# maxjiang216/corintho-ai

Hardware: AMD Instinct MI355X
Metric: self-play games/sec at 400 sims/move (higher is better)
Workload: dtype f32(f16x3)

## Files before the change

corintho_ai_amd/csrc/kernels.h:

```cpp
#pragma once
#include "mcts.h"

CO_CONST int32_t CO_SPACE_SYM[8][16] = CO_SPACE_SYM_INIT;
CO_CONST int32_t CO_MOVE_SYM[8][96] = CO_MOVE_SYM_INIT;

#ifdef CO_EMU
#define CO_K3_WAVES 1
#define CO_K3_WAVE_IN_BLOCK 0
#define CO_K3_BOUNDS
#else
#define CO_K3_BOUNDS __launch_bounds__(CO_K3_WPB * 64)
#define CO_K3_WAVES CO_K3_WPB
#define CO_K3_WAVE_IN_BLOCK (CO_K3_WPB > 1 ? __builtin_amdgcn_readfirstlane((int)(threadIdx.x >> 6)) : 0)
#endif
CO_K3_BOUNDS CO_KERNEL co_k_mcts_step(EngineParams P) {
  const int i = CO_BLOCK_IDX * CO_K3_WAVES + CO_K3_WAVE_IN_BLOCK;
  const int g = P.pool_lo + i;
  if (i < P.pool_n && g < P.num_games) co_mcts_step_wave(P, g);
}

CO_DEV int co_game_active(const EngineParams &P, int g, const GameCtl &gc, int tp) {
  if (gc.done) return 0;
  if (P.pcfg) return tp == CO_TO_PLAY_EVERY_MODEL || P.pcfg[2 * g + gc.to_play].model_id == tp;
  if (tp == 0 || tp == 1) return gc.to_play == (tp + gc.parity) % 2;
  return 1;
}

CO_KERNEL co_k_scan(EngineParams P) {
  int G = P.num_games;
  const int tp = P.arena_state ? P.arena_state[P.scan_phase == 0 ? CO_AS_NEXT : CO_AS_MODEL] : P.to_play;
  int chunk = (G + CO_WAVE - 1) / CO_WAVE;
  LV(int, csum);
  LV(int, nd);
  LV(int, er);
  FOR_LANES {
    int s = 0, notdone = 0, err = 0;
    for (int i = 0; i < chunk; ++i) {
      int g = lane * chunk + i;
      if (g < G) {
        GameCtl gc = P.games[g];
        if (co_game_active(P, g, gc, tp)) s += gc.n_pending;
        notdone += !gc.done;
        err |= gc.error;
      }
    }
    L(csum) = s;
    L(nd) = notdone;
    L(er) = err != 0;
  }
  int not_done = WAVE_SUM_I32(nd);
  int any_error = WAVE_BALLOT(er) != 0;
  WAVE_SHARED(int, cbase, CO_WAVE + 1);
  FOR_LANES { cbase[lane + 1] = L(csum); }
  WAVE_SYNC();
  int run = 0;
  LV(int, mybase);
  FOR_LANES { L(mybase) = 0; }
  for (int l = 0; l < CO_WAVE; ++l) {
    int v = cbase[l + 1];
    FOR_LANES {
      if (lane == l) L(mybase) = run;
    }
    run += v;
  }
  FOR_LANES {
    int s = L(mybase);
    for (int i = 0; i < chunk; ++i) {
      int g = lane * chunk + i;
      if (g < G) {
        GameCtl gc = P.games[g];
        P.req_offset[g] = s;
        if (co_game_active(P, g, gc, tp)) s += gc.n_pending;
      }
    }
    if (lane == 0 && P.read_offset) {
      int offset = 0;
      P.read_offset[0] = 0;
      for (int i = 1; i < G; ++i) {
        if (co_game_active(P, i, P.games[i], tp)) offset += P.games[i - 1].n_pending;
        P.read_offset[i] = offset;
      }
    }
    if (lane == 0) {
      P.req_offset[G] = run;
      P.all_done[0] = not_done == 0;
      if (P.ctl) {
        P.ctl[CO_CTL_ROWS] = run;
        P.ctl[CO_CTL_ALL_DONE] = not_done == 0;
        P.ctl[CO_CTL_ANY_ERROR] = any_error;
        P.ctl[CO_CTL_NOT_DONE] = not_done;
      }
      if (P.row_counter && (!P.arena_state || P.scan_phase == 1)) P.row_counter[0] += (unsigned long long)run;
      if (P.arena_state) {
        if (P.scan_phase == 0) {
          P.arena_state[CO_AS_MODEL] = tp;
        } else {
          P.arena_state[CO_AS_ROWS + (tp == 0 ? 1 : 0)] = run;
          P.arena_state[CO_AS_ROWS + (tp == 0 ? 0 : 1)] = 0;
          if (not_done != 0 && run == 0) {
            P.arena_state[CO_AS_NEXT] = 1 - tp;
            P.arena_state[CO_AS_EMPTY] += 1;
          } else {
            P.arena_state[CO_AS_NEXT] = tp;
            P.arena_state[CO_AS_EMPTY] = 0;
          }
        }
      }
    }
  }
}

CO_KERNEL co_k_compact(EngineParams P) {
  int g = CO_BLOCK_IDX;
  if (g >= P.num_games) return;
  GameCtl gc = P.games[g];
  if (!co_game_active(P, g, gc, P.arena_state ? P.arena_state[CO_AS_MODEL] : P.to_play)) return;
  int n = gc.n_pending;
  const float *src = P.req + (size_t)g * P.searches_per_eval * CO_STATE_STRIDE;
  float *dst = P.nn_in + (size_t)P.req_offset[g] * CO_STATE_STRIDE;
  int total = n * CO_STATE_STRIDE;
  FOR_LANES {
    for (int i = lane; i < total; i += CO_WAVE) dst[i] = src[i];
  }
  if (P.nn_in70) {
    float *d70 = P.nn_in70 + (size_t)P.req_offset[g] * CO_GAME_STATE_SIZE;
    int t70 = n * CO_GAME_STATE_SIZE;
    FOR_LANES {
      for (int i = lane; i < t70; i += CO_WAVE) d70[i] = src[(i / CO_GAME_STATE_SIZE) * CO_STATE_STRIDE + i % CO_GAME_STATE_SIZE];
    }
  }
}

CO_KERNEL co_k_expand_rows(const float *in70, float *out80, int rows, int nblocks) {
  FOR_LANES {
    int total = rows * CO_STATE_STRIDE;
    for (int i = CO_BLOCK_IDX * CO_WAVE + lane; i < total; i += CO_WAVE * nblocks) {
      int r = i / CO_STATE_STRIDE, c = i % CO_STATE_STRIDE;
      out80[i] = c < CO_GAME_STATE_SIZE ? in70[(size_t)r * CO_GAME_STATE_SIZE + c] : 0.0f;
    }
  }
}

#define CO_HOST_ROWS_FLOAT ((CO_BLOCK_IDX * CO_WAVES_PER_BLOCK + CO_WAVE_IN_BLOCK) * CO_WAVE + lane)
CO_KERNEL co_k_host_rows_out(const float *req, const int32_t *in_idx, const uint32_t *count, int cap_rows, float *out70) {
  const uint32_t have = count[0];
  const int rows = (int)(have < (uint32_t)cap_rows ? have : (uint32_t)cap_rows);
  const int total = cap_rows * CO_GAME_STATE_SIZE;
  FOR_LANES {
    const int e = CO_HOST_ROWS_FLOAT;
    if (e < total) {
      const int r = e / CO_GAME_STATE_SIZE, c = e - r * CO_GAME_STATE_SIZE;
      out70[e] = r < rows ? req[(size_t)(in_idx ? in_idx[r] : r) * CO_STATE_STRIDE + c] : 0.0f;
    }
  }
}
CO_KERNEL co_k_host_rows_in(const float *evals, const float *probs, const int32_t *out_idx, const uint32_t *count, int rows,
                            float *d_eval, float *d_probs, int eval_stride, int probs_stride) {
  const uint32_t have = count ? count[0] : (uint32_t)rows;
  const int total = (int)(have < (uint32_t)rows ? have : (uint32_t)rows) * (1 + CO_NUM_MOVES);
  FOR_LANES {
    const int e = CO_HOST_ROWS_FLOAT;
    if (e < total) {
      const int r = e / (1 + CO_NUM_MOVES), c = e - r * (1 + CO_NUM_MOVES);
      const size_t o = (size_t)(out_idx ? out_idx[r] : r);
      if (c == 0) d_eval[o * (size_t)eval_stride] = evals[r];
      else d_probs[o * (size_t)probs_stride + c - 1] = probs[(size_t)r * CO_NUM_MOVES + c - 1];
    }
  }
}

CO_KERNEL co_k_write_samples(EngineParams P, int n_games, const int32_t *sample_offset, const int32_t *meta, float *game_states,
                             float *eval_samples, float *prob_samples) {
  int g = CO_BLOCK_IDX;
  if (g >= n_games) return;
  const int n = meta[g] & 255, result = meta[g] >> 8;
  size_t off = (size_t)sample_offset[g];
  const float *smp = P.samples + (size_t)g * CO_MAX_PLIES * CO_SAMPLE_FLOATS;
  for (int i = n - 1; i >= 0; --i) {
    const float evaluation = co_sample_outcome(result, n, i);
    const float *st = smp + (size_t)i * CO_SAMPLE_FLOATS;
    const float *pol = st + CO_GAME_STATE_SIZE;
    for (int k = 0; k < CO_NUM_SYMMETRIES; ++k) {
      float *gs = game_states + ((off + i) * CO_NUM_SYMMETRIES + k) * CO_GAME_STATE_SIZE;
      float *ps = prob_samples + ((off + i) * CO_NUM_SYMMETRIES + k) * CO_NUM_MOVES;
      FOR_LANES {
        gs[lane] = st[CO_SPACE_SYM[k][lane / 4] * 4 + lane % 4];
        if (lane < CO_GAME_STATE_SIZE - 64) gs[64 + lane] = st[64 + lane];
        ps[lane] = pol[CO_MOVE_SYM[k][lane]];
        if (lane < CO_NUM_MOVES - 64) ps[64 + lane] = pol[CO_MOVE_SYM[k][64 + lane]];
        if (lane == 0) eval_samples[(off + i) * CO_NUM_SYMMETRIES + k] = evaluation;
      }
    }
  }
}

CO_KERNEL co_k_pack_samples(EngineParams P, int n_games, const int32_t *sample_offset, const int32_t *meta, float *state_policy,
                            float *outcome) {
  int g = CO_BLOCK_IDX;
  if (g >= n_games) return;
  const int n = meta[g] & 255, result = meta[g] >> 8;
  size_t off = (size_t)sample_offset[g];
  const float *smp = P.samples + (size_t)g * CO_MAX_PLIES * CO_SAMPLE_FLOATS;
  int total = n * CO_SAMPLE_FLOATS;
  FOR_LANES {
    for (int i = lane; i < total; i += CO_WAVE) state_policy[off * CO_SAMPLE_FLOATS + i] = smp[i];
    for (int i = lane; i < n; i += CO_WAVE) outcome[off + i] = co_sample_outcome(result, n, i);
  }
}

CO_KERNEL co_k_rules_batch(const uint64_t *boards, const uint32_t *metas, int n, uint32_t *masks, int32_t *lines) {
  int i = CO_BLOCK_IDX;
  if (i >= n) return;
  uint32_t lm[3];
  CoLanes K;
  co_lanes_init(K);
  int l = co_legal_moves(boards[i], metas[i], lm, K);
  FOR_LANES {
    if (lane < 3) masks[i * 3 + lane] = lm[lane];
    if (lane == 0) lines[i] = l;
  }
}

CO_KERNEL co_k_domove_batch(uint64_t *boards, uint32_t *metas, const int32_t *moves, int n, float *states) {
  int i = CO_BLOCK_IDX;
  if (i >= n) return;
  uint64_t b = boards[i];
  uint32_t m = metas[i];
  CoLanes K;
  co_lanes_init(K);
  if (moves[i] >= 0) co_do_move(&b, &m, moves[i], K);
  WAVE_SYNC();
  FOR_LANES {
    if (lane == 0) {
      boards[i] = b;
      metas[i] = m;
    }
  }
  co_write_state(b, m, states + (size_t)i * CO_STATE_STRIDE);
}

CO_KERNEL co_k_rules_rows(uint64_t *boards, uint32_t *metas, const int32_t *moves, int n, uint32_t *masks) {
  const int base = CO_BLOCK_IDX * 4;
  LV(uint32_t, blo);
  LV(uint32_t, bhi);
  LV(uint32_t, mt);
  LV(int, on);
  FOR_LANES {
    const int i = base + (lane >> 4);
    L(on) = i < n;
    uint64_t b = L(on) ? boards[i] : 0ull;
    uint32_t m = L(on) ? metas[i] : 0u;
    if (L(on) && moves[i] >= 0) co_do_move_lane(&b, &m, moves[i]);
    L(blo) = (uint32_t)b;
    L(bhi) = (uint32_t)(b >> 32);
    L(mt) = m;
  }
  LV(uint32_t, o0);
  LV(uint32_t, o1);
  LV(uint32_t, o2);
  WG_SHARED(uint32_t, lb, CO_LB_WORDS);
  co_line_breakers_to_lds(lb);
  LV(int, lines);
  co_legal_moves_rows(blo, bhi, mt, on, o0, o1, o2, lines, lb);
  FOR_LANES {
    const int i = base + (lane >> 4);
    if (L(on) && (lane & 15) == 0) {
      boards[i] = (uint64_t)L(blo) | ((uint64_t)L(bhi) << 32);
      metas[i] = L(mt);
      masks[i * 3 + 0] = L(o0);
      masks[i * 3 + 1] = L(o1);
      masks[i * 3 + 2] = L(o2);
    }
  }
}

CO_KERNEL co_k_rng_draw(uint32_t *mt, int32_t *idx_io, int n, int chunk, uint32_t *out) {
  int idx = idx_io[0];
  int done = 0;
  while (done < n) {
    int cnt = n - done < chunk ? n - done : chunk;
    LV(uint32_t, r);
    CO_MT_DRAW(mt, idx, cnt, r);
    FOR_LANES {
      if (lane < cnt) out[done + lane] = L(r);
    }
    done += cnt;
  }
  FOR_LANES {
    if (lane == 0) idx_io[0] = idx;
  }
}

CO_KERNEL co_k_fp_probe(const float *in, int n, float *out) {
  FOR_LANES {
    int i = CO_BLOCK_IDX * CO_WAVE + lane;
    if (i < n) {
      const float *x = in + (size_t)i * 8;
      float c_puct = x[0], visits = x[1], eval = x[2], p9 = x[3], denom = x[4], cv = x[5], sum = x[6], eps = x[7];
      float v_sqrt = (float)((double)c_puct * co_sqrt_f64((double)visits));
      float prob = p9 * denom;
      float pv = prob * v_sqrt;
      int icv = (int)cv;
      double a, b;
      if ((float)icv == cv && icv >= 1 && icv < 32768) {
        a = co_div_small(-(double)eval, cv);
        b = co_div_small((double)pv, cv + 1.0f);
      } else {
        a = -1.0 * (double)eval / (double)cv;
        b = (double)pv / ((double)cv + 1.0);
      }
      float one_minus = (float)1 - eps;
      float *o = out + (size_t)i * 8;
      o[0] = v_sqrt;
      o[1] = (float)(a + b);
      o[2] = pv;
      o[3] = (float)(1.0 / (double)sum * (double)one_minus);
      o[4] = (float)(1.0 / (double)sum * (double)eps);
      o[5] = 511.0f / sum;
      o[6] = (float)(1.0 / (double)(float)(int)cv);
      float xq = p9 * (511.0f / sum);
      float fl = __builtin_truncf(xq);
      int q = (int)fl;
      if (xq - fl >= 0.5f) q += 1;
      o[7] = (float)q;
    }
  }
}
```

corintho_ai_amd/csrc/pools.h:

```cpp
#pragma once
#include <algorithm>
#include <string>
#include <vector>

#include "host.h"
#include "kernels.h"

#define CO_MAX_POOLS 4
#define CO_POOL_POLL 16

struct RunStats {
  double mcts_ms = 0, nn_ms = 0, pack_ms = 0;
  int64_t mcts_launches = 0, nn_launches = 0, nn_rows = 0;
  double mcts_timed_ms = 0, nn_timed_ms = 0, pack_timed_ms = 0;
  int64_t timed_launches = 0, nn_timed_rows = 0;
  int64_t nn_rows_evaluated = 0;
  int64_t steps_cut = 0, step_budget_last = 0;
  int64_t cache_clears = 0;

  void estimate_device_times(bool with_pack) {
    if (timed_launches == 0) return;
    mcts_ms = mcts_timed_ms * (double)mcts_launches / (double)timed_launches;
    nn_ms = nn_timed_ms * (double)nn_launches / (double)timed_launches;
    if (with_pack) pack_ms = pack_timed_ms * (double)nn_launches / (double)timed_launches;
  }
};

static void launch_mcts_step(const EngineParams &e, int n, rt_stream_t s) {
  RT_LAUNCH(co_k_mcts_step, (n + CO_K3_WAVES - 1) / CO_K3_WAVES, CO_WAVE * CO_K3_WAVES, s, e);
}

struct CacheTable {
  DevBuf<uint32_t> hdr;
  DevBuf<float> val;
  DevBuf<uint32_t> done;
  size_t entries = 0;

  void create(int eval_cache, int R, int spe, rt_stream_t s) {
    size_t want = (size_t)R * 8192, n = 1;
    while (n < want) n <<= 1;
    const size_t per = 16 + CO_CACHE_VAL_FLOATS * 4;
    while (n > 1024 && n * per > rt_mem_free() / 6) n >>= 1;
    if (eval_cache > 0) {
      n = (size_t)1 << (eval_cache < 6 ? 6 : eval_cache > 30 ? 30 : eval_cache);
      if (n * per > rt_mem_free() / 2)
        throw CaError(CA_ERR_ARG, "ca_config.eval_cache: a table of 2^" + std::to_string(eval_cache) +
                                          " entries does not fit in the free device memory");
    }
    entries = n;
    hdr.alloc(n * 4, s);
    val.alloc((n + (size_t)R * spe) * CO_CACHE_VAL_FLOATS, s);
    done.alloc(CO_MAX_POOLS, s);
  }
  void release() {
    hdr.release();
    val.release();
    done.release();
    entries = 0;
  }
  void empty(rt_stream_t s, bool new_generation) {
    rt_memset(hdr.p, 0, entries * 16, s);
    if (new_generation) rt_memset(done.p, 0, 4 * CO_MAX_POOLS, s);
  }
};

struct Pool {
  Stream st;
  int lo = 0, n = 0, row_base = 0;
  bool finished = false;
  int idle = 0;
  int running = 0;
  Event ev[2][4];
  Event polled[2];
  int launched[2] = {0, 0};
  int word_iter[2] = {0, 0};
  int first_start = 0;
  int timed[2] = {0, 0};
  struct Seen {
    unsigned long long pack;
    unsigned long long cuts;
    uint32_t evaluated;
  };
  Pinned<Seen> seen;
  unsigned long long cuts_seen = 0;
  DevBuf<int32_t> in_idx, out_idx;
  DevBuf<uint32_t> count;
  DevBuf<unsigned long long> totals;
  EvalCache cache = {};
  double c_inserted_est = 0;
  Event quiet;

  void create(int p, int npools, int R, int spe) {
    st.create();
    lo = (int)((int64_t)R * p / npools);
    n = (int)((int64_t)R * (p + 1) / npools) - lo;
    row_base = lo * spe;
    for (int w = 0; w < 2; ++w) {
      for (auto &e : ev[w]) e.create();
      polled[w].create();
    }
    seen.alloc(2);
    quiet.create();
  }

  void attach(const CacheTable &table, int p, int spe) {
    const size_t rows = (size_t)n * spe;
    in_idx.alloc(rows, st);
    out_idx.alloc(rows, st);
    count.alloc(2 * CO_CACHE_COUNT_STRIDE, st);
    totals.alloc(CO_CACHE_TOTALS, st);
    cache.hdr = table.hdr.p;
    cache.val = table.val.p;
    cache.mask = (uint32_t)(table.entries - 1);
    cache.scratch_base = (uint32_t)row_base;
    cache.pool_bits = (uint32_t)p << CO_CACHE_POOL_SHIFT;
    cache.done = table.done.p;
    cache.in_idx = in_idx.p;
    cache.out_idx = out_idx.p;
    cache.count = count.p;
    cache.totals = totals.p;
    rt_sync(st);
  }

  void begin_run(unsigned long long cuts, int first) {
    cuts_seen = cuts;
    finished = false;
    running = n;
    idle = 0;
    launched[0] = launched[1] = 0;
    timed[0] = timed[1] = 0;
    word_iter[0] = word_iter[1] = 0;
    first_start = first;
  }
};

struct FusedRun {
  CacheTable table;
  std::vector<Pool> pools;
  bool cache_clean = false;
  bool host_stepped = false;

  EngineParams run_params;
  unsigned long long *work_counter = nullptr;
  float *nn_eval = nullptr, *nn_probs = nullptr;
  CoNet *net = nullptr;
  RunStats *stats = nullptr;
  rt_stream_t stream = {};
  int npools = 0, spe = 0;
  static constexpr int poll = CO_POOL_POLL;
  int32_t iteration = 0;
  int window = 0, in_window = 0, parity = 0;
  long long guard_from = -1;
  std::string failure;

  void create(int n, int R, int eval_cache) {
    pools.clear();
    table.release();
    pools.resize(n);
    for (int p = 0; p < n; ++p) {
      Pool &q = pools[p];
      q.create(p, n, R, spe);
      if (eval_cache >= 0) {
        if (p == 0) table.create(eval_cache, R, spe, q.st);
        q.attach(table, p, spe);
      }
    }
    cache_clean = true;
  }
  void release() {
    pools.clear();
    table.release();
  }

  std::vector<unsigned long long> read_work_counters() {
    std::vector<unsigned long long> wc((size_t)CO_WC_WORDS * CO_MAX_POOLS);
    rt_d2h(wc.data(), work_counter, wc.size() * 8, stream);
    rt_sync(stream);
    return wc;
  }

  bool begin(bool mid_generation) {
    const bool cache_clean_now = table.entries && !cache_clean;
    if (cache_clean_now) {
      table.empty(pools[0].st, true);
      for (auto &q : pools) {
        if (!mid_generation) {
          rt_memset(q.count.p, 0, 2 * CO_CACHE_COUNT_STRIDE * 4, q.st);
          rt_memset(q.totals.p, 0, CO_CACHE_TOTALS * 8, q.st);
        }
        rt_sync(q.st);
        q.c_inserted_est = 0;
      }
      cache_clean = true;
    }
    const std::vector<unsigned long long> wc = read_work_counters();
    const EngineParams &P = run_params;
    for (auto &q : pools)
      q.begin_run(wc[CO_WC_WORDS * (&q - &pools[0]) + CO_WC_CUTS], P.stagger_div > 0 ? (P.game_base + q.lo) / P.stagger_div : 0);
    return cache_clean_now;
  }

  void collect(Pool &q, int parity) {
    if (!q.launched[parity]) return;
    rt_event_sync(q.polled[parity]);
    const Pool::Seen &w = q.seen[parity];
    const uint32_t evaluated = q.cache.hdr ? w.evaluated : co_pack_rows(w.pack);
    q.running = (int)co_pack_running(w.pack);
    const bool holding = w.cuts != q.cuts_seen;
    q.cuts_seen = w.cuts;
    if (q.timed[parity]) {
      stats->mcts_timed_ms += rt_event_elapsed_ms(q.ev[parity][0], q.ev[parity][1]);
      stats->pack_timed_ms += rt_event_elapsed_ms(q.ev[parity][1], q.ev[parity][2]);
      stats->nn_timed_ms += rt_event_elapsed_ms(q.ev[parity][2], q.ev[parity][3]);
      stats->nn_timed_rows += (int64_t)evaluated;
      q.c_inserted_est += (double)evaluated * q.launched[parity];
      ++stats->timed_launches;
      q.timed[parity] = 0;
    }
    q.launched[parity] = 0;
    q.finished = q.running == 0;
    if (!q.finished && co_pack_rows(w.pack) == 0 && !holding) {
      if (q.word_iter[parity] > q.first_start && ++q.idle > 16) failure = "No requests during training";
    } else {
      q.idle = 0;
    }
  }

  bool cache_empty_when_half_full() {
    if (!table.entries) return false;
    double taken = 0;
    for (auto &q : pools) taken += q.c_inserted_est;
    if (taken > 0.5 * (double)table.entries) {
      for (int p = 1; p < npools; ++p) {
        rt_event_record(pools[p].quiet, pools[p].st);
        rt_stream_wait(pools[0].st, pools[p].quiet);
      }
      table.empty(pools[0].st, false);
      rt_event_record(pools[0].quiet, pools[0].st);
      for (int p = 1; p < npools; ++p) rt_stream_wait(pools[p].st, pools[0].quiet);
      for (auto &q : pools) q.c_inserted_est = 0;
      ++stats->cache_clears;
      return true;
    }
    return false;
  }

  void queue_iteration(int p, bool emptied, bool timed) {
    Pool &q = pools[p];
    if (q.finished) return;
    EngineParams pp = run_params;
    pp.defer_handover = !host_stepped && q.running * 2 > q.n ? 1 : 0;
    pp.pool_lo = q.lo;
    pp.pool_n = q.n;
    pp.pool_row_base = q.row_base;
    pp.pack_counter = run_params.pack_counter + CO_PACK_STRIDE * p;
    pp.work_counter = work_counter + (size_t)CO_WC_WORDS * p;
    pp.cache = q.cache;
    pp.cache.no_claim = emptied ? 1u : 0u;
    if (emptied) guard_from = iteration;
    pp.cache.guard_pools = 0u;
    if (guard_from >= 0 && iteration <= guard_from + 2 * poll + 1) {
      pp.cache.guard_from = (uint32_t)guard_from;
      for (int p2 = 0; p2 < npools; ++p2)
        if (p2 != p && !pools[p2].finished) pp.cache.guard_pools |= 1u << p2;
    }
    const int cap_rows = (q.running < q.n ? (q.running > 0 ? q.running : 1) : q.n) * spe;
    Event *e = q.ev[parity];
    if (timed) rt_event_record(e[0], q.st);
    launch_mcts_step(pp, q.n, q.st);
    if (timed) rt_event_record(e[1], q.st);
    if (timed) rt_event_record(e[2], q.st);
    CoNetIO io;
    io.alone = npools == 1;
    io.row_base = q.row_base;
    const int32_t *d_rows;
    float *d_eval, *d_probs;
    if (q.cache.hdr) {
      io.in_idx = q.cache.in_idx;
      io.out_idx = q.cache.out_idx;
      io.eval_stride = CO_CACHE_VAL_FLOATS;
      io.probs_stride = CO_CACHE_VAL_FLOATS;
      d_rows = (const int32_t *)(q.cache.count + CO_CACHE_COUNT_STRIDE * (iteration & 1));
      d_eval = q.cache.val;
      d_probs = q.cache.val + 4;
    } else {
      io.in_idx = run_params.row_idx + q.row_base;
      d_rows = (const int32_t *)(pp.pack_counter + (iteration & 1));
      d_eval = nn_eval + q.row_base;
      d_probs = nn_probs + (size_t)q.row_base * CO_NUM_MOVES;
    }
    net->forward(run_params.req, cap_rows, d_rows, d_eval, d_probs, q.st, io);
    if (timed) rt_event_record(e[3], q.st);
    if (timed) q.timed[parity] = 1;
    q.launched[parity] = in_window + 1;
    ++stats->mcts_launches;
    ++stats->nn_launches;
  }

  int64_t run(const EngineParams &params, CoNet *network, int n, int eval_cache, bool mid_generation, int64_t max_iterations) {
    run_params = params;
    run_params.fused_pack = 1;
    net = network;
    spe = params.searches_per_eval;
    npools = n;
    if ((int)pools.size() != npools) create(npools, params.num_games, eval_cache);
    const bool cache_clean_now = begin(mid_generation);
    rt_sync(stream);
    iteration = params.iteration;
    int64_t it = 0;
    in_window = 0, window = 0;
    bool all_finished = false;
    failure.clear();
    bool emptied_before_resuming = cache_clean_now && mid_generation;
    guard_from = -1;
    while (!all_finished && (max_iterations <= 0 || it < max_iterations)) {
      parity = window & 1;
      bool emptied = emptied_before_resuming;
      emptied_before_resuming = false;
      if (cache_empty_when_half_full()) emptied = true;
      run_params.iteration = iteration;
      for (int p = 0; p < npools; ++p)
        queue_iteration(p, emptied, in_window == poll - 1 || (max_iterations > 0 && it + 1 == max_iterations));
      if (net->callback_failed()) break;
      const int counter_slot = iteration & 1;
      ++iteration;
      ++it;
      ++in_window;
      if (in_window == poll || (max_iterations > 0 && it == max_iterations)) {
        for (auto &q : pools) {
          if (q.finished) continue;
          const size_t p = &q - &pools[0];
          Pool::Seen &w = q.seen[parity];
          rt_d2h(&w.pack, run_params.pack_counter + CO_PACK_STRIDE * p + counter_slot, 8, q.st);
          if (q.cache.hdr) rt_d2h(&w.evaluated, q.cache.count + CO_CACHE_COUNT_STRIDE * counter_slot, 4, q.st);
          rt_d2h(&w.cuts, work_counter + (size_t)CO_WC_WORDS * p + CO_WC_CUTS, 8, q.st);
          q.word_iter[parity] = iteration - 1;
          rt_event_record(q.polled[parity], q.st);
        }
        all_finished = true;
        for (auto &q : pools) {
          if (!q.finished) collect(q, parity ^ 1);
          if (!q.finished) all_finished = false;
        }
        in_window = 0;
        ++window;
        if (!failure.empty()) break;
      }
    }
    for (auto &q : pools) {
      rt_sync(q.st);
      for (int w = 0; w < 2; ++w) collect(q, (window + w) & 1);
    }
    return it;
  }

  int64_t rows_evaluated() {
    int64_t rows = 0;
    for (auto &q : pools) {
      unsigned long long tot = 0;
      uint32_t cnt[2 * CO_CACHE_COUNT_STRIDE] = {0};
      rt_d2h(&tot, q.totals.p, 8, q.st);
      rt_d2h(cnt, q.count.p, sizeof cnt, q.st);
      rt_sync(q.st);
      rows += (int64_t)tot + cnt[0] + cnt[CO_CACHE_COUNT_STRIDE];
    }
    return rows;
  }
  void budget_stats() {
    const std::vector<unsigned long long> wc = read_work_counters();
    stats->steps_cut = 0;
    for (size_t p = 0; p < pools.size(); ++p) stats->steps_cut += (int64_t)wc[CO_WC_WORDS * p + CO_WC_CUTS];
    stats->step_budget_last = run_params.step_budget > 0
                                  ? run_params.step_budget
                                  : (int64_t)std::max(wc[CO_WC_BUDGET], wc[CO_WC_BUDGET + 1]) / CO_STEP_UNITS_PER_CONFIG_UNIT;
  }
};
```

corintho_ai_amd/csrc/search_group.h:

```cpp
#pragma once
#include "engine_defs.h"
#include "rules.h"
#include "wave.h"
#include "search_state.h"
#include "search_tree.h"
#include "search_eval.h"
#include "search_puct.h"

#define CO_SB_PE_ONE 96
#define CO_SB_PE_TWO 40
#define CO_SB_DEPTH 12
#define CO_SB_AT(j, lv) ((j) * CO_SB_DEPTH + (lv))
#define CO_SB_SLOT_AT(j, lv) ((j) * (CO_SB_DEPTH + 1) + (lv))

#if defined(CO_SB_STATS) && defined(CO_EMU)
extern unsigned long long co_sb_stats[32];
extern unsigned long long co_sb_ply[8][8];
#define CO_SBS(i, v) __atomic_fetch_add(&co_sb_stats[i], (unsigned long long)(v), __ATOMIC_RELAXED)
#define CO_SBP(w, i, v) __atomic_fetch_add(&co_sb_ply[(w).gc.plies / 4 > 7 ? 7 : (w).gc.plies / 4][i], (unsigned long long)(v), __ATOMIC_RELAXED)
#else
#define CO_SBS(i, v) ((void)0)
#define CO_SBP(w, i, v) ((void)0)
#endif

CO_DEV int co_search_rows(CoWave &w, CoTree &t, CoRoot &rc, int m) {
  uint4 *A = t.A;
  WAVE_SHARED(uint32_t, sb_block, CO_SB * CO_SB_DEPTH);
  WAVE_SHARED(uint32_t, sb_slot, CO_SB * (CO_SB_DEPTH + 1));
  WAVE_SHARED(uint4, sb_cs, CO_SB * CO_SB_DEPTH);
  WAVE_SHARED(uint4, sb_hand, CO_SB * 2);
  WAVE_SHARED(uint4, sb_leaf, CO_SB * 2);
  WAVE_SHARED(int, sb_kn, CO_SB);
  FOR_LANES_HOT {
    if (lane < CO_SB) sb_kn[lane] = -1;
  }
  WAVE_SYNC();
  int bad = m;
  uint32_t shX = t.tc.root;
  uint32_t shown = rc.h1.x;
  uint4 shh0 = rc.h0;
  int lev0 = 0;
  {
    int n0 = (int)CO_META_NEDGES(rc.h0.z);
    float denom0 = co_u2f(rc.h1.y);
    LV(uint4, ev);
    FOR_LANES_HOT { L(ev) = rc.ev[lane]; }
    uint4 rcs = rc.cs;
    LV(double, ea);
    LV(double, er);
    LV(float, ecv1);
    LV(float, eprob);
    LV(int, emode);
    LV(float, vsl);
    for (;;) {
      const int msel = bad < m ? bad : m;
      uint32_t same_slot = CO_NONE;
      uint4 first_bs = make_uint4(0u, 0u, 0u, 0u);
      {
        const int v0 = co_slot_visits(rcs);
        FOR_LANES_HOT {
          const uint4 s = L(ev);
          const int r = CO_SLOT_RESULT(s);
          const int has_child = s.x != CO_NONE;
          const int drawn = (r == CO_RESULT_DRAW) | (r == CO_DEDUCED_DRAW);
          const int searchable = ((r == CO_RESULT_NONE) | drawn) & !CO_SLOT_ALL_VISITED_BIT(s);
          const int vis = co_slot_visits(s);
          const float cv = (float)(vis > 0 ? vis : 1);
          L(eprob) = (float)CO_SLOT_PRIOR_Q(s) * denom0;
          L(ea) = co_div_small(-(double)co_u2f(s.y), cv);
          L(ecv1) = cv + 1.0f;
          L(er) = co_recip_small(L(ecv1));
          L(emode) = !has_child ? 0 : !searchable ? 3 : drawn ? 2 : 1;
          L(vsl) = co_vsqrt(w.c_puct, v0 + (lane < CO_SB ? lane : 0));
        }
      }
      for (int j = 0; j < msel; ++j) {
        CO_SBS(10, 1);
        CO_PROF_ADD(w, 23, 1ull);
        CO_STEP_WORK(w, 1);
        const float v_sqrt = WAVE_BCAST(vsl, j);
        LV(float, u);
        FOR_LANES_HOT {
          const float pv = L(eprob) * v_sqrt;
          const double bq = co_div_with((double)pv, L(ecv1), L(er));
          const float uv = (float)(L(ea) + bq);
          const int md = L(emode);
          const float uu = md == 1 ? uv : md == 3 ? CO_NEG_INF : pv;
          L(u) = lane < n0 ? uu : CO_NEG_INF;
        }
        const float mx = WAVE_MAX_F32(u);
        rcs = co_slot_pass(rcs);
        if (!(mx > CO_NEG_INF)) {
          CO_SBS(3, 1);
          bad = j;
          const uint32_t xo = shown;
          const int lv = lev0;
          FOR_LANES_HOT {
            if (lane == 0) {
              sb_slot[CO_SB_SLOT_AT(j, lv)] = xo;
              sb_cs[CO_SB_AT(j, lv)] = rcs;
              sb_kn[j] = lv;
            }
          }
          break;
        }
        LV(int, hit);
        FOR_LANES_HOT { L(hit) = (L(u) == mx); }
        const int le = co_ffs64(WAVE_BALLOT(hit)) - 1;
        const uint4 bs = WAVE_BCAST(ev, le);
        if (bs.x != CO_NONE && co_res_terminal(co_slot_result(bs))) {
          CO_SBS(4, 1);
          bad = j;
          break;
        }
        const uint32_t child_slot = CO_NODE_EDGE(shX, (uint32_t)le);
        const uint4 nv = bs.x == CO_NONE ? CO_SLOT_BORN(bs) : co_slot_pass(bs);
        if (j == 0) {
          same_slot = bs.x == CO_NONE ? 0u : child_slot;
          first_bs = bs;
        } else if (child_slot != same_slot) {
          same_slot = 0u;
        }
        const uint32_t xb = shX, xo = shown;
        const int lv = lev0;
        FOR_LANES_HOT {
          if (lane == le) {
            L(ev) = nv;
            if (L(emode) == 0) {
              L(emode) = 3;
            } else {
              L(ea) = co_div_with(-(double)co_u2f(nv.y), L(ecv1), L(er));
              L(ecv1) = L(ecv1) + 1.0f;
              L(er) = co_recip_small(L(ecv1));
            }
          }
          if (lane == 0) {
            sb_block[CO_SB_AT(j, lv)] = xb;
            sb_slot[CO_SB_SLOT_AT(j, lv)] = xo;
            sb_slot[CO_SB_SLOT_AT(j, lv) + 1] = child_slot;
            sb_cs[CO_SB_AT(j, lv)] = rcs;
            sb_hand[2 * j] = make_uint4(bs.x, child_slot, bs.z, 0u);
            sb_hand[2 * j + 1] = bs;
          }
        }
      }
      WAVE_SYNC();
      const int left = bad < m ? bad : m;
      if (left < 2 || same_slot == 0u || same_slot == CO_NONE || lev0 + 3 >= CO_SB_DEPTH) break;
      CO_SBS(20, 1);
      shX = first_bs.x;
      shown = same_slot;
      rcs = first_bs;
      ++lev0;
      CO_SBS(9, 1);
      shh0 = co_load_unit(A, shX);
      denom0 = co_u2f(co_load_unit(A, CO_NODE_INFO(shX)).y);
      {
        const uint32_t e0 = CO_NODE_EDGE0(shX);
        FOR_LANES_HOT { L(ev) = A[e0 + lane]; }
      }
      n0 = (int)CO_META_NEDGES(shh0.z);
      if (n0 > CO_WAVE) {
        CO_SBS(5, 1);
        bad = 0;
        break;
      }
    }
  }
  CO_PH(28);
  LV(uint32_t, X);
  LV(uint32_t, slot);
  LV(uint4, cs);
  LV(int, act);
  LV(int, leafD);
  {
    const int nsel = bad < m ? bad : m;
    const uint4 rh0 = shh0;
    const uint32_t root = shX;
    FOR_LANES_HOT {
      const int r = lane >> 4;
      const uint4 h = sb_hand[2 * r], c = sb_hand[2 * r + 1];
      const int valid = r < nsel;
      const int isnew = valid && h.x == CO_NONE;
      L(X) = h.x;
      L(slot) = h.y;
      L(cs) = c;
      L(act) = valid && !isnew;
      L(leafD) = isnew ? lev0 + 1 : 0;
      if (isnew && (lane & 15) == 0) {
        sb_leaf[2 * r] = make_uint4(rh0.x, rh0.y, rh0.z, root);
        sb_leaf[2 * r + 1] = make_uint4(CO_SLOT_MP(h.z), h.y, 0u, 0u);
      }
    }
  }
  for (int lev = lev0 + 1;; ++lev) {
    if (!WAVE_BALLOT(act)) break;
    CO_SBS(9, 1);
    if (lev + 1 >= CO_SB_DEPTH) {
      const int fr = (co_ffs64(WAVE_BALLOT(act)) - 1) >> 4;
      CO_SBS(6, 1);
      if (fr < bad) bad = fr;
      break;
    }
    {
      const uint64_t am = WAVE_BALLOT(act);
      const int a0 = (int)(am & 1ull), a1 = (int)((am >> 16) & 1ull), a2 = (int)((am >> 32) & 1ull), a3 = (int)((am >> 48) & 1ull);
      if (a0 + a1 + a2 + a3 <= 2) {
        CO_SBS(20 + (a0 + a1 + a2 + a3), 1);
        const int r0 = a0 ? 0 : a1 ? 1 : a2 ? 2 : 3;
        const int r1 = a0 + a1 + a2 + a3 < 2 ? -1 : (a3 ? 3 : a2 ? 2 : 1);
        uint32_t wx[2], ws[2];
        uint4 wc[2], wh[2];
        uint32_t wd[2];
        LV(uint4, we[2]);
        int wr[2] = {r0, r1};
#pragma unroll
        for (int i = 0; i < 2; ++i) {
          const int r = wr[i] < 0 ? r0 : wr[i];
          wx[i] = WAVE_BCAST(X, 16 * r);
          ws[i] = WAVE_BCAST(slot, 16 * r);
          wc[i] = WAVE_BCAST(cs, 16 * r);
        }
#pragma unroll
        for (int i = 0; i < 2; ++i) {
          wh[i] = co_load_unit(A, wx[i]);
          wd[i] = co_load_unit(A, CO_NODE_INFO(wx[i])).y;
          const uint32_t e0 = CO_NODE_EDGE0(wx[i]);
          FOR_LANES_HOT { L(we[i]) = A[e0 + lane]; }
        }
        float wvs[2];
#pragma unroll
        for (int i = 0; i < 2; ++i) {
          wvs[i] = co_vsqrt(w.c_puct, co_slot_visits(wc[i]));
          CO_OPAQUE_V(wvs[i]);
        }
        CO_PH_MEM(11);
        uint32_t pX = CO_NONE;
        int pe = -1;
        uint4 pv = make_uint4(0u, 0u, 0u, 0u);
#pragma unroll
        for (int i = 0; i < 2; ++i) {
          const int r = wr[i];
          if (r < 0 || r >= bad) continue;
          CO_SBS(10, 1);
          CO_PROF_ADD(w, 23, 1ull);
          CO_STEP_WORK(w, 1);
          const int n = (int)CO_META_NEDGES(wh[i].z);
          int gone = 0;
          int le = 0;
          uint4 bs = make_uint4(0u, 0u, 0u, 0u);
          if (n > CO_WAVE) {
            CO_SBS(5, 1);
            gone = 1;
          } else {
            const float denom = co_u2f(wd[i]);
            const float v_sqrt = wvs[i];
            LV(float, u);
            FOR_LANES_HOT {
              uint4 sl = L(we[i]);
              if (pe >= 0 && pX == wx[i] && lane == pe) {
                sl = pv;
                CO_SBS(11, 1);
              }
              L(we[i]) = sl;
              const float uu = co_puct_u(sl, denom, v_sqrt);
              L(u) = lane < n ? uu : CO_NEG_INF;
            }
            const float mx = WAVE_MAX_F32(u);
            wc[i] = co_slot_pass(wc[i]);
            if (!(mx > CO_NEG_INF)) {
              CO_SBS(3, 1);
              gone = 1;
              const uint32_t xs = ws[i];
              const uint4 xc = wc[i];
              FOR_LANES_HOT {
                if (lane == 0) {
                  sb_slot[CO_SB_SLOT_AT(r, lev)] = xs;
                  sb_cs[CO_SB_AT(r, lev)] = xc;
                  sb_kn[r] = lev;
                }
              }
            } else {
              LV(int, hit);
              FOR_LANES_HOT { L(hit) = (L(u) == mx); }
              le = co_ffs64(WAVE_BALLOT(hit)) - 1;
              bs = WAVE_BCAST(we[i], le);
              if (bs.x != CO_NONE && co_res_terminal(co_slot_result(bs))) {
                CO_SBS(4, 1);
                gone = 1;
              }
            }
          }
          if (gone) {
            if (r < bad) bad = r;
            FOR_LANES_HOT {
              if ((lane >> 4) >= r) L(act) = 0;
            }
            continue;
          }
          const uint32_t child_slot = CO_NODE_EDGE(wx[i], (uint32_t)le);
          const int isnew = bs.x == CO_NONE;
          pX = wx[i];
          pe = le;
          pv = isnew ? CO_SLOT_BORN(bs) : co_slot_pass(bs);
          const uint32_t xb = wx[i], xs = ws[i];
          const uint4 xc = wc[i], xh = wh[i];
          FOR_LANES_HOT {
            if (lane == 0) {
              sb_block[CO_SB_AT(r, lev)] = xb;
              sb_slot[CO_SB_SLOT_AT(r, lev)] = xs;
              sb_slot[CO_SB_SLOT_AT(r, lev) + 1] = child_slot;
              sb_cs[CO_SB_AT(r, lev)] = xc;
              if (isnew) {
                sb_leaf[2 * r] = make_uint4(xh.x, xh.y, xh.z, xb);
                sb_leaf[2 * r + 1] = make_uint4(CO_SLOT_MP(bs.z), child_slot, 0u, 0u);
              }
            }
            if ((lane >> 4) == r) {
              if (isnew) {
                L(leafD) = lev + 1;
                L(act) = 0;
              } else {
                L(X) = bs.x;
                L(slot) = child_slot;
                L(cs) = bs;
              }
            }
          }
        }
        WAVE_SYNC();
        CO_PH(8);
        continue;
      }
    }
    CO_SBS(23, 1);
    LV(uint4, h0);
    LV(uint32_t, dnb);
    LV(uint4, e0);
    LV(uint4, e1);
    LV(uint4, e2);
    LV(uint4, e3);
    FOR_LANES_HOT {
      if (L(act)) {
        const uint32_t b = L(X);
        const uint32_t c = CO_NODE_EDGE(b, (uint32_t)(lane & 15));
        L(h0) = A[CO_NODE_HDR(b)];
        L(dnb) = A[CO_NODE_INFO(b)].y;
        L(e0) = A[c];
        L(e1) = A[c + 16u];
        L(e2) = A[c + 32u];
        L(e3) = A[c + 48u];
      }
    }
    LV(float, vs);
    FOR_LANES_HOT {
      L(vs) = co_vsqrt(w.c_puct, co_slot_visits(L(cs)));
      CO_OPAQUE_V(L(vs));
    }
    CO_PH_MEM(11);
    LV(int, todo);
    LV(int, wide);
    FOR_LANES_HOT {
      L(wide) = L(act) && (int)CO_META_NEDGES(L(h0).z) > CO_WAVE;
      L(todo) = L(act) && !L(wide);
    }
    {
      const uint64_t wm = WAVE_BALLOT(wide);
      if (wm) {
        const int fr = (co_ffs64(wm) - 1) >> 4;
        CO_SBS(5, 1);
        if (fr < bad) bad = fr;
      }
    }
    for (;;) {
      FOR_LANES_HOT {
        if ((lane >> 4) >= bad) {
          L(todo) = 0;
          L(act) = 0;
        }
      }
      const uint64_t tm = WAVE_BALLOT(todo);
      if (!tm) break;
      CO_SBS(24, 1);
      CO_STEP_WORK(w, 2);
      const uint32_t x0 = WAVE_BCAST(X, 0), x1 = WAVE_BCAST(X, 16), x2 = WAVE_BCAST(X, 32);
      const int t0 = (int)(tm & 1ull), t1 = (int)((tm >> 16) & 1ull), t2 = (int)((tm >> 32) & 1ull);
      LV(int, ready);
      LV(float, bu);
      LV(uint32_t, be);
      LV(uint32_t, bx);
      LV(uint32_t, by);
      LV(uint32_t, bz);
      LV(uint32_t, bw);
      FOR_LANES_HOT {
        const int r = lane >> 4;
        const int blocked = (r > 0 && t0 && x0 == L(X)) || (r > 1 && t1 && x1 == L(X)) || (r > 2 && t2 && x2 == L(X));
        L(ready) = L(todo) && !blocked;
        L(bu) = CO_NEG_INF;
        L(be) = 255u;
        L(bx) = L(by) = L(bz) = L(bw) = 0u;
        if (L(ready)) {
          CO_SBS(10, (lane & 15) == 0);
          CO_PROF_ADD(w, 23, 0ull);
        }
      }
#pragma unroll
      for (int k = 0; k < 4; ++k) {
        LV(int, more);
        FOR_LANES_HOT { L(more) = L(ready) && (int)CO_META_NEDGES(L(h0).z) > 16 * k; }
        if (!WAVE_BALLOT(more)) break;
        FOR_LANES_HOT {
          const uint4 sl = k == 0 ? L(e0) : k == 1 ? L(e1) : k == 2 ? L(e2) : L(e3);
          const int e = 16 * k + (lane & 15);
          float uu = co_puct_u(sl, co_u2f(L(dnb)), L(vs));
          uu = (L(ready) && e < (int)CO_META_NEDGES(L(h0).z)) ? uu : CO_NEG_INF;
          if (uu > L(bu)) {
            L(bu) = uu;
            L(be) = (uint32_t)e;
            L(bx) = sl.x;
            L(by) = sl.y;
            L(bz) = sl.z;
            L(bw) = sl.w;
          }
        }
      }
      LV(float, mx);
      ROW_MAX_F32(mx, bu);
      LV(uint32_t, cand);
      FOR_LANES_HOT { L(cand) = (L(bu) == L(mx) && L(mx) > CO_NEG_INF) ? L(be) : 255u; }
      LV(uint32_t, emin);
      ROW_MIN_U32(emin, cand);
      LV(int, col);
      FOR_LANES_HOT { L(col) = (int)(L(emin) & 15u); }
      ROW_SHFL_U32(bx, bx, col);
      ROW_SHFL_U32(by, by, col);
      ROW_SHFL_U32(bz, bz, col);
      ROW_SHFL_U32(bw, bw, col);
      LV(int, isbad);
      LV(int, fin);
      LV(uint32_t, pX);
      LV(uint4, nv);
      FOR_LANES_HOT {
        L(isbad) = 0;
        L(fin) = L(ready);
        L(pX) = L(X);
        L(nv) = make_uint4(0u, 0u, 0u, 0u);
        if (L(ready)) {
          const int r = lane >> 4;
          const uint4 bs = make_uint4(L(bx), L(by), L(bz), L(bw));
          const int none = L(emin) == 255u;
          const int isnew = bs.x == CO_NONE;
          const int term = !isnew && co_res_terminal(co_slot_result(bs));
          L(cs) = co_slot_pass(L(cs));
          L(isbad) = none || term;
          const uint32_t child_slot = CO_NODE_EDGE(L(X), L(emin));
          if (!L(isbad)) {
            if ((lane & 15) == 0) {
              sb_block[CO_SB_AT(r, lev)] = L(X);
              sb_slot[CO_SB_SLOT_AT(r, lev)] = L(slot);
              sb_slot[CO_SB_SLOT_AT(r, lev) + 1] = child_slot;
              sb_cs[CO_SB_AT(r, lev)] = L(cs);
            }
            if (isnew) {
              L(nv) = CO_SLOT_BORN(bs);
              L(leafD) = lev + 1;
              if ((lane & 15) == 0) {
                sb_leaf[2 * r] = make_uint4(L(h0).x, L(h0).y, L(h0).z, L(X));
                sb_leaf[2 * r + 1] = make_uint4(CO_SLOT_MP(bs.z), child_slot, 0u, 0u);
              }
              L(act) = 0;
            } else {
              L(nv) = co_slot_pass(bs);
              L(X) = bs.x;
              L(slot) = child_slot;
              L(cs) = bs;
            }
          } else {
            if (none) CO_SBS(3, (lane & 15) == 0);
            else CO_SBS(4, (lane & 15) == 0);
            if (none && (lane & 15) == 0) {
              sb_slot[CO_SB_SLOT_AT(r, lev)] = L(slot);
              sb_cs[CO_SB_AT(r, lev)] = L(cs);
              sb_kn[r] = lev;
            }
            L(act) = 0;
          }
          L(todo) = 0;
        }
      }
      {
        const uint64_t bm = WAVE_BALLOT(isbad);
        if (bm) {
          const int fr = (co_ffs64(bm) - 1) >> 4;
          if (fr < bad) bad = fr;
        }
      }
      const uint64_t fm = WAVE_BALLOT(fin), wm2 = WAVE_BALLOT(todo);
      if (wm2) {
#pragma unroll
        for (int r2 = 0; r2 < CO_SB - 1; ++r2) {
          if (!((fm >> (16 * r2)) & 1ull)) continue;
          const uint32_t px = WAVE_BCAST(pX, 16 * r2);
          const uint32_t pe = WAVE_BCAST(emin, 16 * r2);
          const uint4 pv = WAVE_BCAST(nv, 16 * r2);
          FOR_LANES_HOT {
            if (L(todo) && (lane >> 4) > r2 && L(X) == px && (uint32_t)(lane & 15) == (pe & 15u)) {
              CO_SBS(11, 1);
              const uint32_t k = pe >> 4;
              if (k == 0u) L(e0) = pv;
              else if (k == 1u) L(e1) = pv;
              else if (k == 2u) L(e2) = pv;
              else L(e3) = pv;
            }
          }
        }
      }
    }
    CO_PH(8);
  }
  WAVE_SYNC();
  int nsel = bad < m ? bad : m;
  LV(int, on);
  LV(uint32_t, nb0);
  LV(uint32_t, nb1);
  LV(uint32_t, nmeta);
  LV(uint32_t, l0);
  LV(uint32_t, l1);
  LV(uint32_t, l2);
  LV(int, nl);
  LV(uint32_t, lz);
  LV(uint32_t, lpar);
  LV(uint32_t, lslot);
  LV(uint32_t, lmeta);
  FOR_LANES_HOT {
    L(on) = (lane >> 4) < nsel;
    const uint4 la = sb_leaf[2 * (lane >> 4)], lb = sb_leaf[2 * (lane >> 4) + 1];
    L(lz) = lb.x;
    L(lslot) = lb.y;
    L(lpar) = la.w;
    L(lmeta) = la.z;
    uint64_t b = (uint64_t)la.x | ((uint64_t)la.y << 32);
    uint32_t mm = la.z;
    if (L(on)) co_do_move_lane(&b, &mm, (int)CO_SLOT_MOVE(L(lz)));
    L(nb0) = (uint32_t)b;
    L(nb1) = (uint32_t)(b >> 32);
    L(nmeta) = mm;
  }
  LV(int, lin);
  co_legal_moves_rows(nb0, nb1, nmeta, on, l0, l1, l2, lin, w.lb);
  FOR_LANES_HOT { L(nl) = L(on) ? co_popc32(L(l0)) + co_popc32(L(l1)) + co_popc32(L(l2)) : 0; }
  int term = -1;
  {
    uint32_t used = t.tc.units_used;
    int j = 0;
    for (; j < nsel; ++j) {
      const int n = WAVE_BCAST(nl, 16 * j);
      if (CO_NODE_END(used, n) > t.cap) break;
      if (n == 0) {
        CO_SBS(7, 1);
        term = j;
        break;
      }
      used += CO_NODE_UNITS(n);
    }
    if (j < nsel && term < 0) bad = j;
    nsel = j;
  }
  CO_PH(14);
  int done = nsel;
  if (nsel > 0) {
    const int n0 = WAVE_BCAST(nl, 0), n1 = WAVE_BCAST(nl, 16), n2 = WAVE_BCAST(nl, 32), n3 = WAVE_BCAST(nl, 48);
    const uint32_t base0 = t.tc.units_used;
    const int noise0 = w.noise_words, k0 = w.gc.n_pending;
    const int dl[CO_SB] = {WAVE_BCAST(leafD, 0), WAVE_BCAST(leafD, 16), WAVE_BCAST(leafD, 32), WAVE_BCAST(leafD, 48)};
    FOR_LANES_HOT {
      const int r = lane >> 4, c = lane & 15;
      if (r < nsel && c < L(leafD)) {
        const uint32_t sl = sb_slot[CO_SB_SLOT_AT(r, c)];
        int last = 1;
#pragma unroll
        for (int r2 = 1; r2 < CO_SB; ++r2)
          if (r2 > r && r2 < nsel && c < dl[r2] && sb_slot[CO_SB_SLOT_AT(r2, c)] == sl) last = 0;
        if (last) {
          const uint4 v = sb_cs[CO_SB_AT(r, c)];
          A[sl] = v;
          const uint32_t idx = sl - rc.e0;
          if (idx < rc.ne) rc.ev[idx] = v;
        }
      }
    }
    for (int j = 0; j < nsel; ++j) rc.cs = co_slot_pass(rc.cs);
    CO_PH(9);
    LV(uint32_t, nblk);
    LV(int, noff);
    FOR_LANES_HOT {
      const int r = lane >> 4, c = lane & 15;
      const uint32_t before = (r > 0 ? CO_NODE_UNITS(n0) : 0u) + (r > 1 ? CO_NODE_UNITS(n1) : 0u) + (r > 2 ? CO_NODE_UNITS(n2) : 0u);
      L(nblk) = base0 + before;
      L(noff) = noise0 + (r > 0 ? n0 : 0) + (r > 1 ? n1 : 0) + (r > 2 ? n2 : 0);
      if (r < nsel) {
        const uint32_t b = L(nblk);
        const int depth = (int)CO_META_DEPTH(L(lmeta)) + 1;
        if (c == 0) A[CO_NODE_HDR(b)] = make_uint4(L(nb0), L(nb1), co_meta_make(L(nmeta), depth, L(nl)), L(lpar));
        if (c == 1) A[CO_NODE_INFO(b)] = make_uint4(L(lslot), 0u, 0u, 0u);
        const int c0 = co_popc32(L(l0)), c01 = c0 + co_popc32(L(l1));
#pragma unroll
        for (int q = 0; q < 6; ++q) {
          const int id = 16 * q + c;
          const uint32_t wd = q < 2 ? L(l0) : q < 4 ? L(l1) : L(l2);
          const int bit = id & 31;
          if ((wd >> bit) & 1u) {
            const int rank = (q < 2 ? 0 : q < 4 ? c0 : c01) + co_popc32(wd & ((1u << bit) - 1u));
            A[CO_NODE_EDGE(b, (uint32_t)rank)] = CO_SLOT_EDGE(id);
          }
        }
        if (c == 2) {
          const uint4 v = CO_SLOT_NEW(b, co_f2u(1.0f), L(lz), CO_RESULT_NONE);
          A[L(lslot)] = v;
          const uint32_t idx = L(lslot) - rc.e0;
          if (idx < rc.ne) rc.ev[idx] = v;
        }
      }
    }
    {
      const uint32_t units = CO_NODE_FIXED_UNITS * (uint32_t)nsel + (uint32_t)(n0 + (nsel > 1 ? n1 : 0) + (nsel > 2 ? n2 : 0) + (nsel > 3 ? n3 : 0));
      t.tc.units_used = base0 + units;
      if (t.tc.units_used > t.tc.peak_units) t.tc.peak_units = t.tc.units_used;
      w.gc.nodes += (uint32_t)nsel;
      t.tc.searches_done += nsel;
      w.gc.searches += (uint32_t)nsel;
    }
    CO_PH(15);
    CO_PROF_ADD(w, 24, (unsigned long long)nsel);
    if (w.analyse) {
      for (int j = 0; j < nsel; ++j) {
        const int D = WAVE_BCAST(leafD, 16 * j);
        FOR_LANES_HOT {
          if (lane < D) A[CO_NODE_INFO(sb_block[CO_SB_AT(j, lane)])].z += 1u;
        }
        WAVE_SYNC();
      }
    }
    {
      float *req = w.req;
      uint32_t *pend_leaf = w.pend_leaf, *pend_path = w.pend_path, *pend_n = w.pend_n;
      int32_t *pend_depth = w.pend_depth;
      uint4 *pend_key = w.pend_key;
      FOR_LANES_HOT {
        const int r = lane >> 4, c = lane & 15;
        if (r < nsel) {
          const int k = k0 + r;
          const uint64_t b = (uint64_t)L(nb0) | ((uint64_t)L(nb1) << 32);
          uint4 *row = (uint4 *)(req + (size_t)k * CO_STATE_STRIDE);
          const uint32_t nib = (uint32_t)(b >> (4 * c)) & 15u;
          const uint32_t one = co_f2u(1.0f);
          row[c] = make_uint4((nib & 1u) ? one : 0u, (nib & 2u) ? one : 0u, (nib & 4u) ? one : 0u, (nib & 8u) ? one : 0u);
          const uint32_t pcs = L(nmeta) & 0x3FFFFu;
          const uint32_t rot = CO_META_TO_PLAY(L(nmeta)) ? ((pcs >> 9) | (pcs << 9)) & 0x3FFFFu : pcs;
          if (c < 4) {
            uint32_t f[4];
#pragma unroll
            for (int i = 0; i < 4; ++i) {
              const int x = 4 * c + i;
              f[i] = x < 6 ? co_f2u((float)((rot >> (3 * x)) & 7u) * 0.25f) : 0u;
            }
            row[16 + c] = make_uint4(f[0], f[1], f[2], f[3]);
          }
          if (c == 4) {
            pend_leaf[k] = L(nblk);
            pend_depth[k] = L(leafD);
          }
          if (c >= 5 && c < 9) pend_n[4 * k + (c - 5)] = c == 5 ? (((uint32_t)L(noff) << 8) | (uint32_t)L(nl)) : c == 6 ? L(l0) : c == 7 ? L(l1) : L(l2);
          if (c == 9 && pend_key) pend_key[k] = make_uint4(L(nb0), L(nb1), rot | 0x80000000u, 0u);
          if (c <= L(leafD)) pend_path[(size_t)k * CO_PATH_MAX + c] = sb_slot[CO_SB_SLOT_AT(r, c)];
        }
      }
      w.gc.n_pending = k0 + nsel;
      w.noise_words = noise0 + n0 + (nsel > 1 ? n1 : 0) + (nsel > 2 ? n2 : 0) + (nsel > 3 ? n3 : 0);
    }
    WAVE_SYNC();
    CO_PH(17);
  }
  if (term >= 0) {
    const int j = term;
    const int D = WAVE_BCAST(leafD, 16 * j);
    const uint64_t board = (uint64_t)WAVE_BCAST(nb0, 16 * j) | ((uint64_t)WAVE_BCAST(nb1, 16 * j) << 32);
    const uint32_t meta = WAVE_BCAST(nmeta, 16 * j), z = WAVE_BCAST(lz, 16 * j), parent = WAVE_BCAST(lpar, 16 * j);
    const uint32_t child_slot = WAVE_BCAST(lslot, 16 * j);
    const int depth = (int)CO_META_DEPTH(WAVE_BCAST(lmeta, 16 * j)) + 1;
    const int res = WAVE_BCAST(lin, 16 * j) ? CO_RESULT_LOSS : CO_RESULT_DRAW;
    uint32_t *pslot = &sb_slot[CO_SB_SLOT_AT(j, 0)];
    uint32_t *pblock = &sb_block[CO_SB_AT(j, 0)];
    ++t.tc.searches_done;
    w.gc.searches++;
    FOR_LANES_HOT {
      if (lane < D) {
        const uint32_t sl = pslot[lane];
        const uint4 v = sb_cs[CO_SB_AT(j, lane)];
        A[sl] = v;
        const uint32_t idx = sl - rc.e0;
        if (idx < rc.ne) rc.ev[idx] = v;
      }
    }
    WAVE_SYNC();
    const uint32_t none[3] = {0u, 0u, 0u};
    const uint32_t nb = co_emit_node(w, t, board, meta, depth, parent, child_slot, none, 0, res);
    if (nb != CO_NONE) {
      if (w.analyse) {
        FOR_LANES_HOT {
          if (lane < D) A[CO_NODE_INFO(pblock[lane])].z += 1u;
        }
        WAVE_SYNC();
      }
      const float cur_eval = res == CO_RESULT_DRAW ? 0.0f : -1.0f;
      co_store_slot(A, child_slot, CO_SLOT_NEW(nb, co_f2u(cur_eval), z, res), rc);
      co_propagate_terminal(t, pblock, pslot, D);
      FOR_LANES_HOT {
        if (lane < D) {
          int kk = D - lane;
          float ce = ((kk - 1) & 1) ? (float)((double)cur_eval * -1.0) : cur_eval;
          float add = (float)((double)ce - 1.0);
          uint4 s = A[pslot[lane]];
          s.y = co_f2u(co_u2f(s.y) + add);
          A[pslot[lane]] = s;
        }
      }
      WAVE_SYNC();
      CO_PROF_ADD(w, 5, 1ull);
    }
    rc.valid = 0;
    CO_PH(12);
  }
  int dead_end = 0;
  if (term < 0 && done < m && done == bad) {
    WAVE_SYNC();
    const int D = sb_kn[bad];
    if (D >= 0) {
      const int j = bad;
      FOR_LANES_HOT {
        if (lane <= D) {
          uint4 v = sb_cs[CO_SB_AT(j, lane)];
          if (lane == D) v = co_slot_set_all_visited(v, 1);
          v = co_slot_set_visits(v, co_slot_visits(v) - 1);
          v.y = co_f2u(co_u2f(v.y) - 1.0f);
          A[sb_slot[CO_SB_SLOT_AT(j, lane)]] = v;
        }
      }
      WAVE_SYNC();
      rc.valid = 0;
      dead_end = 1;
    }
  }
  CO_SBS(0, 1);
  CO_SBS(1, m);
  CO_SBS(2, done);
  CO_SBP(w, 0, 1);
  CO_SBP(w, 1, m);
  CO_SBP(w, 2, done);
  CO_SBP(w, 3, term >= 0);
  CO_SBP(w, 4, term < 0 && !dead_end && done < m);
  CO_SBS(12 + done, 1);
  CO_PROF_ADD(w, 5, (unsigned long long)done);
  return done | (term >= 0 || dead_end ? 0x100 : 0) | (term < 0 && !dead_end && done < m ? 0x200 : 0);
}
```

corintho_ai_amd/csrc/search_iter.h:

```cpp
#pragma once
#include "engine_defs.h"
#include "rules.h"
#include "wave.h"
#include "search_state.h"
#include "search_tree.h"
#include "search_eval.h"
#include "search_puct.h"
#include "search_one.h"
#include "search_group.h"

CO_DEV void co_request_root(CoWave &w, CoTree &t) {
  uint4 *A = t.A;
  uint32_t root = t.tc.root;
  uint4 h0 = co_load_unit(A, root);
  uint4 h1 = co_load_unit(A, CO_NODE_INFO(root));
  WAVE_SHARED(uint32_t, one_path, 1);
  uint32_t self_slot = h1.x;
  FOR_LANES {
    if (lane == 0) one_path[0] = self_slot;
  }
  WAVE_SYNC();
  uint64_t board = (uint64_t)h0.x | ((uint64_t)h0.y << 32);
  uint32_t lm[3];
  co_legal_moves1(board, h0.z, lm);
  co_request(w, board, h0.z, root, (int)CO_META_NEDGES(h0.z), lm, 0, one_path);
}

CO_DEV int co_mc_do_iteration(CoWave &w, CoTree &t, const float *eval, const float *probs) {
  if (t.tc.root == CO_NONE) {
    int res;
    const uint64_t b0 = w.analyse ? ((uint64_t)w.gc.pos_lo | ((uint64_t)w.gc.pos_hi << 32)) : 0ull;
    uint32_t b = co_create_node(w, t, b0, w.analyse ? (w.gc.pos_meta & 0x7FFFFu) : CO_META_START, 0, CO_NONE, CO_NONE, &res);
    if (b == CO_NONE) return 0;
    t.tc.root = b;
    t.tc.searches_done = 1;
    co_request_root(w, t);
    return 0;
  }
  if (t.tc.searches_done == 0) {
    const uint4 rs = co_load_unit(t.A, co_load_unit(t.A, CO_NODE_INFO(t.tc.root)).x);
    if (co_slot_visits(rs) == 1 && co_slot_all_visited(rs)) {
      t.tc.searches_done = 1;
      co_request_root(w, t);
      return 0;
    }
  }
  if (w.gc.n_pending > 0 && !(w.gc.held & 1)) co_receive_eval(w, t, eval, probs);
  w.gc.held = (w.gc.held & 2) | ((w.gc.held & 1) << 1);
  WAVE_SHARED(uint4, root_ev, CO_WAVE);
  CoRoot rc;
  rc.valid = 0;
  rc.hdr = 0;
  rc.ev = root_ev;
  rc.e0 = 0u;
  rc.ne = 0u;
  int pe = w.gc.sb_cap > 0 && w.gc.sb_cap <= 256 ? w.gc.sb_cap : 0;
  for (;;) {
    if (!(w.gc.n_pending < w.spe && t.tc.searches_done < w.max_searches)) break;
    if (!rc.valid) co_root_load(t, rc);

    if (co_res_known(co_slot_result(rc.cs)) || co_slot_all_visited(rc.cs)) break;
    if (w.gc.error) break;
    if ((w.gc.held & 4) && CO_STEP_SPENT(w)) {
      w.gc.held |= 1;
      break;
    }
    CO_PH_MEM(20);
    int counted = 0;
    {
      const int cap = pe > CO_SB_PE_ONE ? 1 : pe > CO_SB_PE_TWO ? 2 : CO_SB;
      int m = w.spe - w.gc.n_pending;
      if (w.max_searches - t.tc.searches_done < m) m = w.max_searches - t.tc.searches_done;
      if (m > cap) m = cap;
      if (m > 1 && (int)CO_META_NEDGES(rc.h0.z) <= CO_WAVE) {
        const int r = co_search_rows(w, t, rc, m);
        w.gc.held |= 4;
        for (int i = 0; i < (r & 0xFF); ++i) pe -= pe >> 3;
        if (r & 0x300) {
          pe += (256 - pe) >> 3;
          counted = 1;
        }
        if (!(r & 0x200)) continue;
      }
    }
    const int pending_before = w.gc.n_pending;
    CO_SBS(8, 1);
    CO_SBP(w, 6, 1);
    co_search(w, t, rc);
    w.gc.held |= 4;
    CO_PROF_ADD(w, 5, 1ull);
    if (!counted) {
      if (w.gc.n_pending > pending_before) pe -= pe >> 3;
      else pe += (256 - pe) >> 3;
    }
  }
  w.gc.sb_cap = pe > 0 ? pe : 0;
  if (w.gc.n_pending != 0 || (w.gc.held & 1)) return 0;
  if (t.tc.searches_done == w.max_searches) return 1;
  const uint4 rs = co_load_unit(t.A, co_load_unit(t.A, CO_NODE_INFO(t.tc.root)).x);
  return co_res_known(co_slot_result(rs));
}
```

corintho_ai_amd/csrc/search_move.h:

```cpp
#pragma once
#include "engine_defs.h"
#include "rules.h"
#include "wave.h"
#include "search_state.h"
#include "search_tree.h"
#include "search_eval.h"
#include "search_iter.h"

CO_DEV void co_move_down(CoTree &t, uint32_t child_block) {
  uint4 h0 = co_load_unit(t.A, child_block);
  h0.w = CO_NONE;
  co_store_unit(t.A, child_block, h0);
  t.tc.root = child_block;
  t.tc.searches_done = 0;
}

CO_DEV void co_reset_tree_to_child(CoWave &w, CoTree &t, int choice) {
  uint4 h0 = co_load_unit(t.A, t.tc.root);
  uint64_t board = (uint64_t)h0.x | ((uint64_t)h0.y << 32);
  uint32_t meta = h0.z;
  int depth = (int)CO_META_DEPTH(meta) + 1;
  co_do_move_lane(&board, &meta, choice);
  int res;
  uint32_t b = co_create_node(w, t, board, meta, depth, CO_NONE, CO_NONE, &res);
  if (b == CO_NONE) return;
  t.tc.root = b;
  t.tc.searches_done = 0;
}

CO_DEV void co_log_put(CoWave &w, int &at, int32_t v) {
  if (at + 1 < CO_LOG_CAP) {
    int32_t *dst = w.log + 1 + at;
    FOR_LANES {
      if (lane == 0) *dst = v;
    }
  }
  ++at;
}
CO_DEV void co_log_commit(CoWave &w, int at) {
  int32_t *dst = w.log;
  FOR_LANES {
    if (lane == 0) *dst = at;
  }
  WAVE_SYNC();
}

CO_DEV void co_log_ply(CoWave &w, CoTree &t, uint4 (&ch)[CO_NUM_MOVES]) {
  uint4 *A = t.A;
  uint32_t node = t.tc.root;
  uint4 h0 = co_load_unit(A, node);
  uint4 h1 = co_load_unit(A, CO_NODE_INFO(node));
  uint4 rs = co_load_unit(A, h1.x);
  int at = w.log[0];
  co_log_put(w, at, 1);
  co_log_put(w, at, w.gc.to_play);
  co_log_put(w, at, (int)CO_META_DEPTH(h0.z));
  co_log_put(w, at, co_slot_visits(rs));
  co_log_put(w, at, co_slot_result(rs));
  co_log_put(w, at, (int32_t)rs.y);
  int depth = (int)CO_META_DEPTH(h0.z);
  for (int level = 0;; ++level) {
    int n = (int)CO_META_NEDGES(h0.z);
    float denom = co_u2f(h1.y);
    WAVE_SYNC();
    for (int base = 0; base < n; base += CO_WAVE) {
      FOR_LANES {
        int e = base + lane;
        if (e < n) ch[e] = A[CO_NODE_EDGE(node, e)];
      }
    }
    WAVE_SYNC();
    if (level == 0) {
      int nc = 0;
      for (int e = 0; e < n; ++e) nc += ch[e].x != CO_NONE;
      co_log_put(w, at, nc);
      for (int e = 0; e < n; ++e) {
        if (ch[e].x == CO_NONE) continue;
        co_log_put(w, at, (int)CO_SLOT_MOVE(ch[e].z));
        co_log_put(w, at, co_slot_visits(ch[e]));
        co_log_put(w, at, (int32_t)ch[e].y);
        co_log_put(w, at, co_slot_result(ch[e]));
        co_log_put(w, at, (int32_t)co_f2u((float)CO_SLOT_PRIOR_Q(ch[e]) * denom));
      }
    }
    int best = -1, max_visits = 0;
    float max_eval = 0.0f;
    for (int e = 0; e < n; ++e) {
      if (ch[e].x == CO_NONE) continue;
      int r = co_slot_result(ch[e]), v = co_slot_visits(ch[e]);
      float ev = co_u2f(ch[e].y);
      if (co_res_lost(r)) {
        best = e;
        break;
      }
      if (v > max_visits || (v == max_visits && ev > max_eval)) {
        best = e;
        max_visits = v;
        max_eval = ev;
      }
    }
    if (best < 0) break;
    ++depth;
    co_log_put(w, at, depth);
    co_log_put(w, at, (int)CO_SLOT_MOVE(ch[best].z));
    co_log_put(w, at, co_slot_visits(ch[best]));
    co_log_put(w, at, co_slot_result(ch[best]));
    co_log_put(w, at, (int32_t)ch[best].y);
    co_log_put(w, at, (int32_t)co_f2u((float)CO_SLOT_PRIOR_Q(ch[best]) * denom));
    node = ch[best].x;
    h0 = co_load_unit(A, node);
    h1 = co_load_unit(A, CO_NODE_INFO(node));
  }
  co_log_put(w, at, -1);
  co_log_commit(w, at);
}

CO_COLD int co_choose_move(CoWave &w, CoTree &t, float *sample) {
  uint4 *A = t.A;
  uint32_t root = t.tc.root;
  uint4 h0 = co_load_unit(A, root);
  uint4 h1 = co_load_unit(A, CO_NODE_INFO(root));
  uint4 rs = co_load_unit(A, h1.x);
  int n = (int)CO_META_NEDGES(h0.z);
  float denom = co_u2f(h1.y);
  int rres = co_slot_result(rs);
  uint64_t board = (uint64_t)h0.x | ((uint64_t)h0.y << 32);
  float *policy = sample ? sample + CO_GAME_STATE_SIZE : (float *)0;
  if (!w.testing) {
    WAVE_SHARED(float, srow, CO_STATE_STRIDE);
    co_write_state(board, h0.z, srow);
    WAVE_SYNC();
    FOR_LANES {
      sample[lane] = srow[lane];
      if (lane < CO_GAME_STATE_SIZE - 64) sample[64 + lane] = srow[64 + lane];
      policy[lane] = 0.0f;
      if (lane < CO_NUM_MOVES - 64) policy[64 + lane] = 0.0f;
    }
    WAVE_SYNC();
  }
  WAVE_SHARED(uint4, ch, CO_NUM_MOVES);
  if (w.log) co_log_ply(w, t, ch);
  for (int base = 0; base < n; base += CO_WAVE) {
    FOR_LANES {
      int e = base + lane;
      if (e < n) ch[e] = A[CO_NODE_EDGE(root, e)];
    }
  }
  WAVE_SYNC();
  if (w.trace_on) {
    co_trace_push(w, w.gc.to_play);
    co_trace_push(w, (int)CO_META_DEPTH(h0.z));
    co_trace_push(w, co_slot_visits(rs));
    co_trace_push(w, rres);
    co_trace_push(w, (int32_t)rs.y);
    int nc = 0;
    for (int e = 0; e < n; ++e) nc += ch[e].x != CO_NONE;
    co_trace_push(w, nc);
    for (int e = 0; e < n; ++e) {
      if (ch[e].x == CO_NONE) continue;
      co_trace_push(w, (int)CO_SLOT_MOVE(ch[e].z));
      co_trace_push(w, co_slot_visits(ch[e]));
      co_trace_push(w, (int32_t)ch[e].y);
      co_trace_push(w, co_slot_result(ch[e]));
      co_trace_push(w, co_slot_all_visited(ch[e]));
    }
  }
  int choice = 0;
  int chosen_e = -1;
  if (co_res_won(rres)) {
    for (int e = 0; e < n; ++e) {
      if (ch[e].x != CO_NONE && co_res_lost(co_slot_result(ch[e]))) {
        choice = (int)CO_SLOT_MOVE(ch[e].z);
        chosen_e = e;
        break;
      }
    }
  } else if (co_res_lost(rres) || co_res_drawn(rres)) {
    int max_visits = 0;
    for (int e = 0; e < n; ++e) {
      if (ch[e].x == CO_NONE) continue;
      int v = co_slot_visits(ch[e]);
      if (v > max_visits && (co_res_lost(rres) || !co_res_won(co_slot_result(ch[e])))) {
        choice = (int)CO_SLOT_MOVE(ch[e].z);
        chosen_e = e;
        max_visits = v;
      }
    }
  } else {
    int32_t max_prob = 0;
    for (int e = 0; e < n; ++e) {
      float p = (float)CO_SLOT_PRIOR_Q(ch[e]) * denom;
      if (p > (float)max_prob) {
        max_prob = (int32_t)p;
        choice = (int)CO_SLOT_MOVE(ch[e].z);
      }
    }
    if ((int)CO_META_DEPTH(h0.z) < 6 && !w.testing) {
      int32_t visits = 0;
      for (int e = 0; e < n; ++e)
        if (ch[e].x != CO_NONE && !co_res_won(co_slot_result(ch[e]))) visits += co_slot_visits(ch[e]);
      float denominator = (float)(1.0 / (double)(float)visits);
      FOR_LANES {
        for (int e = lane; e < n; e += CO_WAVE)
          if (ch[e].x != CO_NONE && !co_res_won(co_slot_result(ch[e])))
            policy[CO_SLOT_MOVE(ch[e].z)] = (float)co_slot_visits(ch[e]) * denominator;
      }
      WAVE_SYNC();
      if (visits == 0) {
        FOR_LANES {
          if (lane == 0) policy[choice] = 1.0f;
        }
        WAVE_SYNC();
        co_reset_tree_to_child(w, t, choice);
        return choice;
      }
      int32_t target = (int32_t)(co_wave_mt_next(w) % (uint32_t)visits);
      int32_t total = 0;
      for (int e = 0; e < n; ++e) {
        if (ch[e].x == CO_NONE || co_res_won(co_slot_result(ch[e]))) continue;
        total += co_slot_visits(ch[e]);
        if (total > target) {
          choice = (int)CO_SLOT_MOVE(ch[e].z);
          chosen_e = e;
          break;
        }
      }
      if (chosen_e < 0) {
        w.gc.error |= CO_ERR_INTERNAL;
        return choice;
      }
      co_move_down(t, ch[chosen_e].x);
      return choice;
    }
    int max_visits = 0;
    float max_eval = 0.0f;
    for (int e = 0; e < n; ++e) {
      if (ch[e].x == CO_NONE) continue;
      int r = co_slot_result(ch[e]);
      if (co_res_won(r)) continue;
      float ev = co_u2f(ch[e].y);
      if (r == CO_RESULT_DRAW || r == CO_DEDUCED_DRAW) ev = 0.0f;
      int v = co_slot_visits(ch[e]);
      if (v > max_visits || (v == max_visits && ev > max_eval)) {
        choice = (int)CO_SLOT_MOVE(ch[e].z);
        chosen_e = e;
        max_visits = v;
        max_eval = ev;
      }
    }
    if (policy) {
      FOR_LANES {
        if (lane == 0) policy[choice] = 1.0f;
      }
      WAVE_SYNC();
    }
    if (max_visits == 0) {
      co_reset_tree_to_child(w, t, choice);
      return choice;
    }
    co_move_down(t, ch[chosen_e].x);
    return choice;
  }
  if (policy) {
    FOR_LANES {
      if (lane == 0) policy[choice] = 1.0f;
    }
    WAVE_SYNC();
  }
  if (chosen_e < 0) {
    w.gc.error |= CO_ERR_INTERNAL;
    return choice;
  }
  co_move_down(t, ch[chosen_e].x);
  return choice;
}

CO_COLD int co_receive_opponent_move(CoWave &w, CoTree &t, int move_choice, uint64_t board, uint32_t meta_game,
                                    int depth) {
  uint4 *A = t.A;
  uint32_t root = t.tc.root;
  int n = (int)CO_META_NEDGES(co_load_unit(A, root).z);
  uint32_t found = CO_NONE;
  for (int base = 0; base < n; base += CO_WAVE) {
    LV(int, hit);
    LV(uint32_t, cb);
    FOR_LANES {
      int e = base + lane;
      L(hit) = 0;
      L(cb) = CO_NONE;
      if (e < n) {
        uint4 s = A[CO_NODE_EDGE(root, e)];
        L(cb) = s.x;
        L(hit) = (s.x != CO_NONE) && ((int)CO_SLOT_MOVE(s.z) == move_choice);
      }
    }
    uint64_t m = WAVE_BALLOT(hit);
    if (m) found = WAVE_BCAST(cb, co_ffs64(m) - 1);
  }
  if (found != CO_NONE) {
    co_move_down(t, found);
    return 0;
  }
  int res;
  uint32_t b = co_create_node(w, t, board, meta_game, depth, CO_NONE, CO_NONE, &res);
  if (b == CO_NONE) return 1;
  t.tc.root = b;
  co_request_root(w, t);
  t.tc.searches_done = 1;
  return 1;
}

CO_DEV void co_use_player(CoWave &w, int p) {
  if (!w.pc) return;
  w.max_searches = w.pc[p].max_searches;
  w.spe = w.pc[p].searches_per_eval;
  w.c_puct = w.pc[p].c_puct;
  w.epsilon = w.pc[p].epsilon;
}

CO_DEV uint32_t co_uniform_below(CoWave &w, uint32_t n) {
  unsigned long long product = (unsigned long long)co_wave_mt_next(w) * (unsigned long long)n;
  uint32_t low = (uint32_t)product;
  if (low < n) {
    uint32_t threshold = (0u - n) % n;
    while (low < threshold) {
      product = (unsigned long long)co_wave_mt_next(w) * (unsigned long long)n;
      low = (uint32_t)product;
    }
  }
  return (uint32_t)(product >> 32);
}

CO_DEV int co_nth_move(const uint32_t lm[3], int k) {
  for (int wd = 0; wd < 3; ++wd) {
    int c = co_popc32(lm[wd]);
    if (k < c) {
      uint32_t m = lm[wd];
      for (int i = 0; i < k; ++i) m &= m - 1u;
      return wd * 32 + co_ffs64((uint64_t)m) - 1;
    }
    k -= c;
  }
  return -1;
}

CO_DEV void co_analyse_finish(CoWave &w, CoTree &t, int choice) {
  uint4 h0 = co_load_unit(t.A, t.tc.root);
  uint4 h1 = co_load_unit(t.A, CO_NODE_INFO(t.tc.root));
  uint4 rs = co_load_unit(t.A, h1.x);
  uint32_t lm[3];
  co_legal_moves1((uint64_t)h0.x | ((uint64_t)h0.y << 32), h0.z, lm);
  uint32_t *out = (uint32_t *)w.req;
  FOR_LANES {
    if (lane == 0) {
      out[0] = (uint32_t)choice;
      out[1] = (uint32_t)co_slot_result(rs);
      out[2] = h1.z + 1u;
      out[3] = rs.y;
      out[4] = lm[0];
      out[5] = lm[1];
      out[6] = lm[2];
      out[7] = 1u;
    }
  }
  WAVE_SYNC();
}
```

corintho_ai_amd/csrc/search_one.h:

```cpp
#pragma once
#include "engine_defs.h"
#include "rules.h"
#include "wave.h"
#include "search_state.h"
#include "search_tree.h"
#include "search_eval.h"
#include "search_puct.h"

CO_COLD2 void co_search(CoWave &w, CoTree &t, CoRoot &rc) {
  uint4 *A = t.A;
  WAVE_SHARED(uint32_t, path_block, CO_PATH_MAX);
  WAVE_SHARED(uint32_t, path_slot, CO_PATH_MAX);
  uint32_t cur = t.tc.root;
  ++t.tc.searches_done;
  w.gc.searches++;
  uint4 h0 = rc.h0;
  uint4 h1 = rc.h1;
  uint32_t cur_slot = h1.x;
  uint4 cs = rc.cs;
  LV(uint4, ev);
  FOR_LANES { L(ev) = rc.ev[lane]; }
  int D = 0;
  int leaf_n = 0;
  uint32_t leaf_lm[3] = {0u, 0u, 0u};
  FOR_LANES {
    if (lane == 0) {
      path_block[0] = cur;
      path_slot[0] = cur_slot;
    }
  }
  WAVE_SYNC();
  CO_PH_MEM(19);
  float v_sqrt_next = co_vsqrt(w.c_puct, co_slot_visits(cs));
  while (!co_res_terminal(co_slot_result(cs))) {
    int n = (int)CO_META_NEDGES(h0.z);
    float denom = co_u2f(h1.y);
    int visits = co_slot_visits(cs);
    const float v_sqrt = v_sqrt_next;
    float best_u = CO_NEG_INF;
    int best_e = -1;
    uint4 best_slot = make_uint4(0, 0, 0, 0);
    for (int base = 0; base < n; base += CO_WAVE) {
      LV(float, u);
      FOR_LANES {
        int e = base + lane;
        float uu = CO_NEG_INF;
        if (base > 0 && e < n) L(ev) = A[CO_NODE_EDGE(cur, e)];
        uu = co_puct_u(L(ev), denom, v_sqrt);
        uu = e < n ? uu : CO_NEG_INF;
        L(u) = uu;
      }
      float mx = WAVE_MAX_F32(u);
      if (mx > best_u) {
        LV(int, hit);
        FOR_LANES { L(hit) = (L(u) == mx); }
        int le = co_ffs64(WAVE_BALLOT(hit)) - 1;
        best_u = mx;
        best_e = base + le;
        best_slot = WAVE_BCAST(ev, le);
      }
    }
    CO_PH(8);
    CO_PROF_ADD(w, 23, 1ull);
    CO_STEP_WORK(w, 1);
    cs = co_slot_set_visits(cs, visits + 1);
    cs.y = co_f2u(co_u2f(cs.y) + 1.0f);
    if (best_e < 0) {
      cs = co_slot_set_all_visited(cs, 1);
      co_store_slot(A, cur_slot, cs, rc);
      FOR_LANES {
        if (lane <= D) {
          uint4 s = A[path_slot[lane]];
          s = co_slot_set_visits(s, co_slot_visits(s) - 1);
          s.y = co_f2u(co_u2f(s.y) - 1.0f);
          A[path_slot[lane]] = s;
        }
      }
      WAVE_SYNC();
      --t.tc.searches_done;
      w.gc.searches--;
      rc.valid = 0;
      return;
    }
    co_store_slot(A, cur_slot, cs, rc);
    if (D == 0) rc.cs = cs;
    if (D + 1 >= CO_PATH_MAX) {
      w.gc.error |= CO_ERR_PATH_TOO_DEEP;
      return;
    }
    uint32_t child_slot = CO_NODE_EDGE(cur, (uint32_t)best_e);
    CO_PH(9);
    if (best_slot.x == CO_NONE) {
      uint64_t board = (uint64_t)h0.x | ((uint64_t)h0.y << 32);
      uint32_t meta = h0.z;
      int move = (int)CO_SLOT_MOVE(best_slot.z);
      co_do_move_lane(&board, &meta, move);
      int res;
      int depth = (int)CO_META_DEPTH(h0.z) + 1;
      CO_PH(16);
      CO_PROF_ADD(w, 24, 1ull);
      uint32_t nb = co_create_node(w, t, board, meta, depth, cur, child_slot, &res, &leaf_n, leaf_lm);
      if (nb == CO_NONE) return;
      if (w.analyse) {
        FOR_LANES {
          if (lane <= D) A[CO_NODE_INFO(path_block[lane])].z += 1u;
        }
        WAVE_SYNC();
      }
      cs = CO_SLOT_NEW(nb, 0u, CO_SLOT_MP(best_slot.z), res);
      cur = nb;
      cur_slot = child_slot;
      h0 = make_uint4((uint32_t)board, (uint32_t)(board >> 32), co_meta_make(meta, depth, 0), 0u);
      ++D;
      FOR_LANES {
        if (lane == 0) {
          path_block[D] = cur;
          path_slot[D] = cur_slot;
        }
      }
      WAVE_SYNC();
      CO_PH(10);
      break;
    }
    cur = best_slot.x;
    cur_slot = child_slot;
    cs = best_slot;
    h0 = co_load_unit(A, cur);
    h1 = co_load_unit(A, CO_NODE_INFO(cur));
    FOR_LANES { L(ev) = A[CO_NODE_EDGE(cur, lane)]; }
    v_sqrt_next = co_vsqrt(w.c_puct, co_slot_visits(cs));
    CO_OPAQUE_V(v_sqrt_next);
    CO_PH_MEM(11);
    ++D;
    FOR_LANES {
      if (lane == 0) {
        path_block[D] = cur;
        path_slot[D] = cur_slot;
      }
    }
    WAVE_SYNC();
  }
  int r = co_slot_result(cs);
  if (co_res_terminal(r)) {
    float cur_eval = co_res_drawn(r) ? 0.0f : -1.0f;
    cs.y = co_f2u(cur_eval);
    co_store_slot(A, cur_slot, cs, rc);
    co_propagate_terminal(t, path_block, path_slot, D);
    FOR_LANES {
      if (lane < D) {
        int kk = D - lane;
        float ce = ((kk - 1) & 1) ? (float)((double)cur_eval * -1.0) : cur_eval;
        float add = (float)((double)ce - 1.0);
        uint4 s = A[path_slot[lane]];
        s.y = co_f2u(co_u2f(s.y) + add);
        A[path_slot[lane]] = s;
      }
    }
    WAVE_SYNC();
    rc.valid = 0;
    CO_PH(12);
  } else {
    cs.y = co_f2u(1.0f);
    co_store_slot(A, cur_slot, cs, rc);
    uint64_t board = (uint64_t)h0.x | ((uint64_t)h0.y << 32);
    co_request(w, board, h0.z, cur, leaf_n, leaf_lm, D, path_slot);
  }
}
```

corintho_ai_amd/csrc/search_state.h:

```cpp
#pragma once
#include "engine_defs.h"
#include "rng.h"
#include "rules.h"
#include "wave.h"

CO_CONST uint32_t CO_GAMMA_BITS[CO_NUM_GAMMA] = CO_GAMMA_BITS_INIT;

#define CO_NEG_INF (-__builtin_huge_valf())

#define CO_NPROF 32
#if defined(CO_PROF) && !defined(CO_EMU)
#define CO_CLK() __builtin_amdgcn_s_memtime()
#define CO_PROF_ADD(w, slot, v) ((w).pacc[slot] += (v))
#define CO_PH(slot)                               \
  do {                                            \
    unsigned long long now_ = CO_CLK();           \
    w.pacc[slot] += now_ - w.tph;                 \
    w.tph = now_;                                 \
  } while (0)
#define CO_PH_MEM(slot)                                               \
  do {                                                                \
    asm volatile("s_waitcnt vmcnt(0) lgkmcnt(0)" ::: "memory");       \
    CO_PH(slot);                                                      \
  } while (0)
#else
#define CO_CLK() 0ull
#define CO_PROF_ADD(w, slot, v) ((void)0)
#define CO_PH(slot) ((void)0)
#define CO_PH_MEM(slot) ((void)0)
#endif

#ifndef CO_EMU
#define CO_STEP_CLOCK() ((uint32_t)__builtin_amdgcn_s_memrealtime())
#define CO_STEP_UNITS_PER_CONFIG_UNIT 100
#define CO_STEP_WORK(w, n) ((void)0)
#define CO_STEP_START(budget) ((int)(CO_STEP_CLOCK() + (uint32_t)(budget)))
#define CO_STEP_SPENT(w) ((int)(CO_STEP_CLOCK() - (uint32_t)(w).work) >= 0)
#define CO_STEP_DONE(w, budget) ((int)(CO_STEP_CLOCK() - ((uint32_t)(w).work - (uint32_t)(budget))))
#else
#define CO_STEP_UNITS_PER_CONFIG_UNIT 1
#define CO_STEP_WORK(w, n) ((w).work += (n))
#define CO_STEP_START(budget) (-(budget))
#define CO_STEP_SPENT(w) ((w).work >= 0)
#define CO_STEP_DONE(w, budget) ((w).work + (budget))
#endif

struct CoTree {
  uint4 *A;
  TreeCtl tc;
  uint32_t cap;
};

struct CoWave {
  int g;
  GameCtl gc;
#if defined(CO_PROF) && !defined(CO_EMU)
  unsigned long long pacc[CO_NPROF], tph;
#endif
  CoTree me, opp;
  uint32_t *mt;
  const uint32_t *gamma;
  const uint32_t *lb;
  int mt_staged;
  uint32_t *mt_stage;
  uint32_t *pend_leaf;
  int32_t *pend_depth;
  uint32_t *pend_path;
  uint32_t *pend_n;
  uint4 *pend_key;
  const float *cval;
  const int32_t *csrc;
  uint32_t *noise_raw;
  int noise_words;
  int work;
  int pre_n, pre_c0;
  uint32_t *pre;
  float *req;
  float *samples;
  int32_t *trace;
  int32_t *log;
  unsigned long long *prof;
  int max_searches, spe, testing, trace_on, defer_handover, analyse, force_choose;
  float c_puct, epsilon;
  const PlayerCfg *pc;
};
```

corintho_ai_amd/csrc/search_step.h:

```cpp
#pragma once
#include "engine_defs.h"
#include "rng.h"
#include "rules.h"
#include "wave.h"
#include "search_state.h"
#include "search_tree.h"
#include "search_eval.h"
#include "search_iter.h"
#include "search_move.h"

CO_DEV int co_game_step(CoWave &w, const float *eval, const float *probs) {
  const float *ev = eval, *pr = probs;
  if (w.gc.resume) {
    w.gc.resume = 0;
    ev = pr = (const float *)0;
  }
  if (w.gc.held & 1) ev = pr = (const float *)0;
  int skip_iteration = (w.pc && w.pc[w.gc.to_play].random)  || w.force_choose;
  int fresh_root = 0;
  for (;;) {
    if (!skip_iteration) {
      int done = co_mc_do_iteration(w, w.me, ev, pr);
      if (w.gc.error) return 0;
      if (fresh_root) return done;
      if (!done) return 0;
    }
    skip_iteration = 0;
    ev = pr = (const float *)0;
    CO_PH(20);
    int p = w.gc.to_play;
    int choice, terminal, tres, depth;
    uint64_t board;
    uint32_t meta;
    if (w.pc && w.pc[p].random) {
      board = (uint64_t)w.gc.pos_lo | ((uint64_t)w.gc.pos_hi << 32);
      meta = w.gc.pos_meta;
      uint32_t lm[3];
      co_legal_moves1(board, meta, lm);
      int n = co_popc32(lm[0]) + co_popc32(lm[1]) + co_popc32(lm[2]);
      choice = co_nth_move(lm, (int)co_uniform_below(w, (uint32_t)n));
      co_trace_push(w, -2);
      co_trace_push(w, choice);
      w.gc.plies++;
      co_do_move_lane(&board, &meta, choice);
      int lines = co_legal_moves1(board, meta, lm);
      terminal = (lm[0] | lm[1] | lm[2]) == 0u;
      tres = lines ? CO_RESULT_LOSS : CO_RESULT_DRAW;
      depth = w.gc.plies;
      if (w.log) {
        int at = w.log[0];
        co_log_put(w, at, 2);
        co_log_put(w, at, choice);
        co_log_put(w, at, (int32_t)(uint32_t)board);
        co_log_put(w, at, (int32_t)(uint32_t)(board >> 32));
        co_log_put(w, at, (int32_t)meta);
        co_log_commit(w, at);
      }
    } else {
      CoTree &me = w.me;
      if (!w.pc) {
        uint4 rs = co_load_unit(me.A, co_load_unit(me.A, CO_NODE_INFO(me.tc.root)).x);
        if (co_res_known(co_slot_result(rs)) && w.gc.mate_turn == 0) w.gc.mate_turn = w.gc.n_samples + 1;
      }
      float *sample = (float *)0;
      if (!w.testing) {
        if (w.gc.n_samples >= CO_MAX_PLIES) {
          w.gc.error |= CO_ERR_TOO_MANY_PLIES;
          return 0;
        }
        sample = w.samples + (size_t)w.gc.n_samples * CO_SAMPLE_FLOATS;
      }
      choice = co_choose_move(w, me, sample);
      if (w.gc.error) return 0;
      if (w.analyse) {
        co_analyse_finish(w, me, choice);
        w.gc.plies++;
        return 1;
      }
      if (!w.testing) w.gc.n_samples++;
      co_trace_push(w, choice);
      w.gc.plies++;
      uint4 h0 = co_load_unit(me.A, me.tc.root);
      uint4 nrs = co_load_unit(me.A, co_load_unit(me.A, CO_NODE_INFO(me.tc.root)).x);
      tres = co_slot_result(nrs);
      terminal = co_res_terminal(tres);
      board = (uint64_t)h0.x | ((uint64_t)h0.y << 32);
      meta = h0.z;
      depth = (int)CO_META_DEPTH(h0.z);
      if (w.log) {
        int at = w.log[0];
        co_log_put(w, at, choice);
        co_log_put(w, at, (int32_t)h0.x);
        co_log_put(w, at, (int32_t)h0.y);
        co_log_put(w, at, (int32_t)meta);
        co_log_commit(w, at);
      }
    }
    if (w.pc) {
      w.gc.pos_lo = (uint32_t)board;
      w.gc.pos_hi = (uint32_t)(board >> 32);
      w.gc.pos_meta = meta & 0x7FFFFu;
    }
    CO_PH_MEM(2);
    if (terminal) {
      if (tres == CO_RESULT_DRAW) w.gc.result = CO_RESULT_DRAW;
      else if (p == 1) w.gc.result = CO_RESULT_LOSS;
      else w.gc.result = CO_RESULT_WIN;
      return 1;
    }
    w.gc.to_play = 1 - p;
    {
      CoTree tmp = w.me;
      w.me = w.opp;
      w.opp = tmp;
    }
    co_use_player(w, 1 - p);
    if (w.pc && w.pc[1 - p].random) {
      skip_iteration = 1;
      continue;
    }
    CoTree &nm = w.me;
    if (nm.tc.root == CO_NONE) {
      int res;
      uint32_t b = co_create_node(w, nm, board, meta, depth, CO_NONE, CO_NONE, &res);
      if (b == CO_NONE) return 0;
      nm.tc.root = b;
      fresh_root = 1;
      continue;
    }
    if (co_receive_opponent_move(w, nm, choice, board, meta, depth)) return 0;
    if (w.defer_handover) {
      w.gc.resume = 1;
      return 0;
    }
  }
}

CO_DEV int co_step_gate(const EngineParams &P, int g, const GameCtl &gc) {
  if (gc.done || gc.error) return 0;
  const int tp = P.arena_state ? P.arena_state[CO_AS_MODEL] : P.to_play;
  if (P.pcfg) {
    if (tp != CO_TO_PLAY_EVERY_MODEL && P.pcfg[2 * g + gc.to_play].model_id != tp) return 0;
  } else if (tp == 0 || tp == 1) {
    if (gc.to_play != (tp + gc.parity) % 2) return 0;
  } else if (P.stagger_div > 0) {
    if ((P.game_base + g) / P.stagger_div > P.iteration) return 2;
  }
  return 1;
}

CO_DEV int co_step_row(const EngineParams &P, int g, const GameCtl &gc) {
  return P.fused_pack ? gc.row_off : P.read_offset ? P.read_offset[g] : P.req_offset[g];
}

CO_DEV uint32_t co_cache_hash(uint32_t k0, uint32_t k1, uint32_t k2) {
  uint32_t h = k0 * 0x9E3779B1u;
  h = (h ^ (h >> 15)) + k1 * 0x85EBCA77u;
  h = (h ^ (h >> 13)) + k2 * 0xC2B2AE3Du;
  h ^= h >> 16;
  h *= 0x27D4EB2Fu;
  return h ^ (h >> 15);
}

CO_DEV void co_cache_resolve(const EngineParams &P, CoWave &w, int g, int n, int row0) {
  const EvalCache &C = P.cache;
  const int par = P.iteration & 1;
  int may_claim = !C.no_claim;
  if (may_claim && C.guard_pools) {
    for (uint32_t p = 0; p < 4u; ++p)
      if (((C.guard_pools >> p) & 1u) && co_atomic_load_u32(C.done + p) <= C.guard_from) may_claim = 0;
  }
  LV(int, slot);
  LV(int, need);
  FOR_LANES {
    int sl = -1, nd = 0;
    if (lane < n) {
      const uint4 key = w.pend_key[lane];
      const uint32_t h = co_cache_hash(key.x, key.y, key.z);
      nd = 1;
      const uint32_t x0 = key.x ^ 0x88888888u, x1 = key.y ^ 0x88888888u;
      const uint32_t mine = key.z | C.pool_bits;
      for (int probe = 0; probe < CO_CACHE_PROBES; ++probe) {
        const uint32_t s = (h + (uint32_t)probe) & C.mask;
        uint32_t *H = C.hdr + (size_t)s * 4;
        uint32_t e0 = co_lane_load_coherent_u32(H + 0), e1 = co_lane_load_coherent_u32(H + 1), e2 = co_lane_load_coherent_u32(H + 2);
        if (e2 == 0u) {
          if (!may_claim) break;
          e2 = co_lane_cas_u32(H + 2, 0u, mine);
          if (e2 == 0u) {
            co_lane_store_coherent_u32(H + 0, x0);
            co_lane_store_coherent_u32(H + 1, x1);
            co_lane_store_coherent_u32(H + 3, (uint32_t)P.iteration + 1u);
            sl = (int)s;
            break;
          }
          if ((e2 & ~CO_CACHE_POOL_MASK) == key.z) {
            e0 = co_lane_load_coherent_u32(H + 0);
            e1 = co_lane_load_coherent_u32(H + 1);
          }
        }
        if ((e2 & ~CO_CACHE_POOL_MASK) == key.z && e0 == x0 && e1 == x1) {
          if ((e2 & CO_CACHE_POOL_MASK) == C.pool_bits) {
            sl = (int)s;
            nd = 0;
          } else {
            const uint32_t stamp = co_lane_load_coherent_u32(H + 3);
            const uint32_t dn = co_lane_load_coherent_u32(C.done + ((e2 & CO_CACHE_POOL_MASK) >> CO_CACHE_POOL_SHIFT));
            if (stamp != 0u && stamp <= dn) {
              sl = (int)s;
              nd = 0;
            }
          }
          break;
        }
      }
    }
    L(slot) = sl;
    L(need) = nd;
  }
  const uint64_t nm = WAVE_BALLOT(need);
  const uint32_t cnt = (uint32_t)co_popc64(nm);
  uint32_t base = 0u;
  if (cnt) base = co_atomic_add_u32(C.count + CO_CACHE_COUNT_STRIDE * par, cnt);
  int32_t *psrc = P.pend_src + (size_t)g * P.searches_per_eval;
  FOR_LANES {
    if (lane < n) {
      int src = L(slot);
      if (L(need)) {
        const uint32_t m = base + (uint32_t)co_popc64(nm & ((1ull << lane) - 1ull));
        if (src < 0) src = (int)(C.mask + 1u + C.scratch_base + m);
        C.in_idx[m] = row0 + lane;
        C.out_idx[m] = src;
      }
      psrc[lane] = src;
    }
  }
}


CO_DEV void co_pool_housekeeping(const EngineParams &P, int g) {
  if (P.fused_pack && g == P.pool_lo) {
    FOR_LANES {
      if (lane == 0) {
        P.pack_counter[(P.iteration + 1) & 1] = 0ull;
        if (P.work_counter) {
          const unsigned long long wc = P.work_counter[(P.iteration + 2) % 3];
          const uint32_t steps = (uint32_t)(wc >> 32), scans = (uint32_t)wc;
          unsigned long long sm = P.work_counter[CO_WC_MEAN + ((P.iteration + 1) & 1)];
          if (steps > 0u) {
            const unsigned long long inst = ((unsigned long long)scans << 8) / steps;
            sm = sm ? (7ull * sm + inst) >> 3 : inst;
          }
          uint32_t b = 0u;
          if (sm > 0ull && P.step_budget_k16 > 0) {
            b = (uint32_t)((sm * (uint32_t)P.step_budget_k16) >> 12);
            if (b < CO_STEP_BUDGET_MIN) b = CO_STEP_BUDGET_MIN;
          }
          P.work_counter[CO_WC_MEAN + (P.iteration & 1)] = sm;
          P.work_counter[CO_WC_BUDGET + (P.iteration & 1)] = (unsigned long long)b;
          P.work_counter[(P.iteration + 1) % 3] = 0ull;
        }
        if (P.cache.hdr) {
          const int op = (P.iteration & 1) ^ 1;
          P.cache.totals[0] += P.cache.count[CO_CACHE_COUNT_STRIDE * op];
          P.cache.count[CO_CACHE_COUNT_STRIDE * op] = 0u;
          co_lane_store_coherent_u32(P.cache.done + (P.cache.pool_bits >> CO_CACHE_POOL_SHIFT), (uint32_t)P.iteration);
        }
      }
    }
  }
}

#define CO_STEP_BUDGET_NONE (1 << 28)
CO_DEV int co_step_budget(const EngineParams &P) {
  if (!(P.fused_pack && !P.testing && !P.analyse && !P.pcfg)) return CO_STEP_BUDGET_NONE;
  int b = P.step_budget * CO_STEP_UNITS_PER_CONFIG_UNIT;
  if (P.step_budget == 0 && P.step_budget_k16 > 0 && P.work_counter) b = (int)(uint32_t)P.work_counter[CO_WC_BUDGET + ((P.iteration + 1) & 1)];
  return b > 0 ? b : CO_STEP_BUDGET_NONE;
}

CO_DEV void co_wave_init(const EngineParams &P, int g, const GameCtl &gc, const TreeCtl &tc0, const TreeCtl &tc1, CoWave &w) {
  w.g = g;
  w.gc = gc;
  {
    const size_t stride = (size_t)P.cap_units + CO_ARENA_PAD;
    const int tm = 2 * g + gc.to_play, to = 2 * g + 1 - gc.to_play;
    w.me.A = P.arena + (size_t)tm * stride;
    w.me.tc = gc.to_play ? tc1 : tc0;
    w.me.cap = P.cap_units;
    w.opp.A = P.arena + (size_t)to * stride;
    w.opp.tc = gc.to_play ? tc0 : tc1;
    w.opp.cap = P.cap_units;
  }
  w.mt = P.rng + (size_t)g * CO_MT_N;
  w.pend_leaf = P.pend_leaf + (size_t)g * P.searches_per_eval;
  w.pend_depth = P.pend_depth + (size_t)g * P.searches_per_eval;
  w.pend_path = P.pend_path + (size_t)g * P.searches_per_eval * CO_PATH_MAX;
  w.pend_n = P.pend_n + (size_t)g * P.searches_per_eval * 4;
  w.pend_key = P.cache.hdr ? P.pend_key + (size_t)g * P.searches_per_eval : (uint4 *)0;
  w.noise_raw = P.noise_raw + (size_t)g * P.searches_per_eval * CO_NUM_MOVES;
  w.noise_words = (gc.held & 1) ? gc.noise_held : 0;
  w.work = CO_STEP_START(co_step_budget(P));
  w.req = P.req + (size_t)g * P.searches_per_eval * CO_STATE_STRIDE;
  w.samples = P.samples ? P.samples + (size_t)gc.gid * CO_MAX_PLIES * CO_SAMPLE_FLOATS : (float *)0;
  w.trace = P.trace ? P.trace + (size_t)gc.gid * CO_TRACE_CAP : (int32_t *)0;
  w.log = (int32_t *)0;
  if (P.log) {
    const int rec = P.log_index ? P.log_index[gc.gid] : gc.gid < P.num_logged ? gc.gid : -1;
    if (rec >= 0) w.log = P.log + (size_t)rec * CO_LOG_CAP;
  }
  w.prof = P.prof ? P.prof + (size_t)g * CO_NPROF : (unsigned long long *)0;
  w.max_searches = P.max_searches;
  w.spe = P.searches_per_eval;
  w.testing = P.testing;
  w.trace_on = P.trace_on && P.trace;
  w.defer_handover = P.defer_handover;
  w.analyse = P.analyse;
  w.force_choose = P.analyse && P.force_choose;
  w.c_puct = P.c_puct;
  w.epsilon = P.epsilon;
  w.pc = P.pcfg ? P.pcfg + 2 * g : (const PlayerCfg *)0;
  co_use_player(w, gc.to_play);
  w.cval = P.cache.hdr ? P.cache.val : (const float *)0;
  w.csrc = P.cache.hdr ? P.pend_src + (size_t)g * P.searches_per_eval : (const int32_t *)0;
}

CO_COLD int co_slot_next_game(const EngineParams &P, CoWave &w) {
  w.gc.done = 1;
  if (!P.results) return 0;
  {
    GameCtl *dst = P.results + w.gc.gid;
    FOR_LANES {
      if (lane == 0) *dst = w.gc;
    }
    WAVE_SYNC();
  }
  const unsigned long long next = co_atomic_add_u64(P.next_game, 1ull);
  if (next >= (unsigned long long)P.total_local) return 0;
  const int gid = (int)next;
  if (w.gc.to_play != 0) {
    CoTree tmp = w.me;
    w.me = w.opp;
    w.opp = tmp;
  }
  GameCtl fresh;
  fresh.to_play = 0; fresh.done = 0; fresh.result = 0; fresh.mate_turn = 0; fresh.n_samples = 0;
  fresh.parity = (P.game_base + gid) % 2; fresh.error = 0; fresh.n_pending = 0; fresh.rng_idx = CO_MT_N;
  fresh.plies = 0; fresh.searches = 0u; fresh.evals = 0u; fresh.nodes = 0u; fresh.trace_len = 0;
  fresh.row_off = 0; fresh.resume = 0; fresh.pos_lo = 0u; fresh.pos_hi = 0u; fresh.pos_meta = CO_META_START;
  fresh.gid = gid;
  fresh.sb_cap = 0;
  fresh.held = 0;
  fresh.noise_held = 0;
  w.gc = fresh;
  w.me.tc.root = CO_NONE; w.me.tc.searches_done = 0; w.me.tc.units_used = 0u;
  w.opp.tc.root = CO_NONE; w.opp.tc.searches_done = 0; w.opp.tc.units_used = 0u;
  w.noise_words = 0;
  w.samples = P.samples ? P.samples + (size_t)gid * CO_MAX_PLIES * CO_SAMPLE_FLOATS : (float *)0;
  w.trace = P.trace ? P.trace + (size_t)gid * CO_TRACE_CAP : (int32_t *)0;
  w.log = (int32_t *)0;
  co_mt_seed(w.mt, P.seeds[gid]);
  w.mt_staged = 0;
  return 1;
}

CO_DEV void co_step_tail(const EngineParams &P, CoWave &w, int g, int done) {
  const int packs = P.fused_pack && !w.gc.done && !w.gc.error;
  unsigned long long old = 0ull;
  CO_PH_MEM(25);
  if (packs && P.work_counter) {
    const int scans = CO_STEP_DONE(w, co_step_budget(P));
    if (scans > 0) co_atomic_add_u64_noret(P.work_counter + P.iteration % 3, ((w.gc.held & 2) ? 0ull : 1ull << 32) | (unsigned long long)scans);
  }
  w.gc.held &= 1;
  if (packs && w.gc.held) {
    co_atomic_add_u64_noret(P.pack_counter + (P.iteration & 1), CO_PACK_ONE_RUNNING);
    if (P.work_counter) co_atomic_add_u64_noret(P.work_counter + CO_WC_CUTS, 1ull);
    w.gc.noise_held = w.noise_words;
    return;
  }
  if (packs) old = co_atomic_add_u64(P.pack_counter + (P.iteration & 1), CO_PACK_ONE_RUNNING | (unsigned long long)w.gc.n_pending);
  CO_PH_MEM(26);
  if (!done && !w.gc.error && w.gc.n_pending > 0) co_capture_noise(w);
  CO_PH_MEM(27);
  if (packs) {
    const int n = w.gc.n_pending;
    const int base = P.pool_row_base + (int)co_pack_rows(old);
    w.gc.row_off = base;
    const int first = g * P.searches_per_eval;
    if (w.pend_key) {
      co_cache_resolve(P, w, g, n, first);
    } else {
      int32_t *ri = P.row_idx + base;
      FOR_LANES {
        if (lane < n) ri[lane] = first + lane;
      }
    }
  }
}

CO_DEV void co_wave_store(const EngineParams &P, const CoWave &w, int g) {
  FOR_LANES {
    if (lane == 0) {
      P.games[g] = w.gc;
      P.trees[2 * g + w.gc.to_play] = w.me.tc;
      P.trees[2 * g + 1 - w.gc.to_play] = w.opp.tc;
    }
  }
}

CO_DEV void co_mcts_step_wave(const EngineParams &P, int g) {
  co_pool_housekeeping(P, g);
  GameCtl gc = P.games[g];
  const TreeCtl tc0 = P.trees[2 * g], tc1 = P.trees[2 * g + 1];
  const int gate = co_step_gate(P, g, gc);
  if (gate != 1) {
    if (gate == 2 && P.fused_pack) co_atomic_add_u64(P.pack_counter + (P.iteration & 1), CO_PACK_ONE_RUNNING);
    return;
  }
  CoWave w;
  WAVE_SHARED(uint32_t, mt_stage, CO_MT_STAGE);
  w.mt_stage = mt_stage;
  WAVE_SHARED(uint32_t, pre_rec, CO_PRE_WORDS);
  w.pre = pre_rec;
  WG_SHARED(uint32_t, lb, CO_LB_WORDS);
  co_line_breakers_to_lds(lb);
  w.lb = lb;
  WG_SHARED(uint32_t, gam, CO_NUM_GAMMA);
  {
    FOR_LANES {
#pragma unroll
      for (int i = 0; i < CO_NUM_GAMMA / CO_WAVE; ++i) gam[i * CO_WAVE + lane] = CO_GAMMA_BITS[i * CO_WAVE + lane];
    }
    WAVE_SYNC();
  }
  w.gamma = gam;
#if defined(CO_PROF) && !defined(CO_EMU)
  const unsigned long long t_wave0 = CO_CLK(), t_real0 = __builtin_amdgcn_s_memrealtime();
  for (int i = 0; i < CO_NPROF; ++i) w.pacc[i] = 0ull;
  w.tph = t_wave0;
#endif
  co_wave_init(P, g, gc, tc0, tc1, w);
  w.pre_n = 0;
  if (w.gc.n_pending > 0 && !(w.gc.held & 1)) co_pending_records(w, 0, w.gc.n_pending < CO_PRE ? w.gc.n_pending : CO_PRE);
  co_mt_stage_load(w.mt, w.mt_stage);
  w.mt_staged = 1;
  CO_PROF_ADD(w, 4, 1ull);
  CO_PH_MEM(22);
  int off = co_step_row(P, g, gc);
  const float *step_eval = P.nn_eval + off, *step_probs = P.nn_probs + (size_t)off * CO_NUM_MOVES;
  int done;
  for (;;) {
    done = co_game_step(w, step_eval, step_probs);
    if (!done) break;
    if (!co_slot_next_game(P, w)) break;
    step_eval = step_probs = (const float *)0;
  }
  CO_PH(20);
  co_step_tail(P, w, g, done);
  CO_PH_MEM(21);
#if defined(CO_PROF) && !defined(CO_EMU)
  w.pacc[7] = CO_CLK() - t_wave0;
  if (w.prof && (threadIdx.x & 63) == 0) {
    for (int i = 0; i < CO_NPROF; ++i) w.prof[i] += w.pacc[i];
    const unsigned long long dt = w.pacc[7];
    unsigned long long *glob = P.prof + (size_t)P.num_games * CO_NPROF;
    if (g == 1) {
      glob[0] += dt;
      glob[1] += __builtin_amdgcn_s_memrealtime() - t_real0;
    }
    atomicMax(glob + 2, dt);
#ifndef CO_PROF_SLOW_FROM
#define CO_PROF_SLOW_FROM 0
#endif
#ifndef CO_PROF_SLOW_CYCLES
#define CO_PROF_SLOW_CYCLES 280000ull
#endif
    if (dt > CO_PROF_SLOW_CYCLES && P.iteration >= CO_PROF_SLOW_FROM) {
      for (int i = 0; i < CO_NPROF; ++i) atomicAdd(glob + 24 + i, w.pacc[i]);
    }
    int bucket = (int)(dt / 50000ull);
    if (bucket > 15) bucket = 15;
    atomicAdd(glob + 4 + bucket, 1ull);
  }
#endif
  co_wave_store(P, w, g);
}
```

corintho_ai_amd/csrc/search_tree.h:

```cpp
#pragma once
#include "engine_defs.h"
#include "rules.h"
#include "wave.h"
#include "search_state.h"

#define CO_NODE_HDR(b) (b)
#define CO_NODE_INFO(b) ((b) + 1u)
#define CO_NODE_EDGE0(b) ((b) + 2u)
#define CO_NODE_EDGE(b, e) (CO_NODE_EDGE0(b) + (e))
#define CO_NODE_END(b, n) CO_NODE_EDGE(b, (uint32_t)(n))
#define CO_NODE_FIXED_UNITS 2u
#define CO_NODE_UNITS(n) (CO_NODE_FIXED_UNITS + (uint32_t)(n))
#define CO_SLOT_MOVE(z) ((z) & 127u)
#define CO_SLOT_PRIOR_Q(s) (((s).z >> 7) & 511u)
#define CO_SLOT_MP(z) ((z) & 0xFFFFu)
#define CO_SLOT_MP_MAKE(id, q) ((uint32_t)(id) | ((uint32_t)((q) & 511) << 7))
#define CO_SLOT_VISITS_SHIFT 16
#define CO_SLOT_ONE_VISIT (1u << CO_SLOT_VISITS_SHIFT)
#define CO_SLOT_RESULT_MASK 0xFFu
#define CO_SLOT_RESULT(s) ((int)((s).w & CO_SLOT_RESULT_MASK))
#define CO_SLOT_ALL_VISITED 0x100u
#define CO_SLOT_ALL_VISITED_BIT(s) (((s).w >> 8) & 1u)
#define CO_SLOT_EDGE(id) make_uint4(CO_NONE, 0u, (uint32_t)(id), 0u)
#define CO_SLOT_NEW(child, eval_bits, mp, res) make_uint4(child, eval_bits, (mp) | CO_SLOT_ONE_VISIT, (uint32_t)(res) | CO_SLOT_ALL_VISITED)
#define CO_SLOT_BORN(bs) make_uint4(0u, co_f2u(1.0f), CO_SLOT_MP((bs).z) | CO_SLOT_ONE_VISIT, CO_SLOT_ALL_VISITED)

CO_DEV int co_slot_visits(uint4 s) { return (int)(int16_t)(s.z >> CO_SLOT_VISITS_SHIFT); }
CO_DEV uint4 co_slot_set_visits(uint4 s, int v) {
  s.z = CO_SLOT_MP(s.z) | ((uint32_t)(uint16_t)(int16_t)v << CO_SLOT_VISITS_SHIFT);
  return s;
}
CO_DEV int co_slot_result(uint4 s) { return CO_SLOT_RESULT(s); }
CO_DEV int co_slot_all_visited(uint4 s) { return (int)CO_SLOT_ALL_VISITED_BIT(s); }
CO_DEV uint4 co_slot_set_result(uint4 s, int r) {
  s.w = (s.w & ~CO_SLOT_RESULT_MASK) | (uint32_t)r;
  return s;
}
CO_DEV uint4 co_slot_set_all_visited(uint4 s, int a) {
  s.w = (s.w & ~CO_SLOT_ALL_VISITED) | ((uint32_t)(a & 1) << 8);
  return s;
}
CO_DEV int co_res_terminal(int r) { return r == CO_RESULT_LOSS || r == CO_RESULT_DRAW; }
CO_DEV int co_res_known(int r) { return r != CO_RESULT_NONE; }
CO_DEV int co_res_won(int r) { return r == CO_DEDUCED_WIN; }
CO_DEV int co_res_lost(int r) { return r == CO_RESULT_LOSS || r == CO_DEDUCED_LOSS; }
CO_DEV int co_res_drawn(int r) { return r == CO_RESULT_DRAW || r == CO_DEDUCED_DRAW; }

CO_DEV uint4 co_load_unit(const uint4 *A, uint32_t off) { return A[off]; }
CO_DEV void co_store_unit(uint4 *A, uint32_t off, uint4 v) {
  FOR_LANES {
    if (lane == 0) A[off] = v;
  }
  WAVE_SYNC();
}

CO_DEV void co_trace_push(CoWave &w, int32_t v) {
  if (!w.trace_on) return;
  if (w.gc.trace_len < CO_TRACE_CAP) {
    int at = w.gc.trace_len;
    FOR_LANES {
      if (lane == 0) w.trace[at] = v;
    }
  }
  w.gc.trace_len++;
}

CO_DEV uint32_t co_emit_node(CoWave &w, CoTree &t, uint64_t board, uint32_t meta_game, int depth, uint32_t parent,
                             uint32_t self_slot, const uint32_t lm[3], int n, int res) {
  const int n01 = co_popc32(lm[0]) + co_popc32(lm[1]);
  uint32_t units = CO_NODE_UNITS(n) + (self_slot == CO_NONE ? 1u : 0u);
  if (t.tc.units_used + units > t.cap) {
    w.gc.error |= CO_ERR_ARENA_FULL;
    return CO_NONE;
  }
  uint32_t b = t.tc.units_used;
  t.tc.units_used += units;
  if (t.tc.units_used > t.tc.peak_units) t.tc.peak_units = t.tc.units_used;
  w.gc.nodes++;
  uint32_t own = self_slot == CO_NONE ? CO_NODE_END(b, n) : self_slot;
  uint32_t meta = co_meta_make(meta_game, depth, n);
  uint4 *A = t.A;
  FOR_LANES {
    if (lane == 0) A[CO_NODE_HDR(b)] = make_uint4((uint32_t)board, (uint32_t)(board >> 32), meta, parent);
    if (lane == 1) A[CO_NODE_INFO(b)] = make_uint4(own, 0u, 0u, 0u);
    if (lane == 2 && self_slot == CO_NONE)
      A[own] = CO_SLOT_NEW(CO_NONE, 0u, 0u, res);
    const uint64_t lm01 = (uint64_t)lm[0] | ((uint64_t)lm[1] << 32);
    if ((lm01 >> lane) & 1ull) A[CO_NODE_EDGE(b, LANE_RANK64(lm01))] = CO_SLOT_EDGE(lane);
    if (((uint64_t)lm[2] >> lane) & 1ull) A[CO_NODE_EDGE(b, n01) + LANE_RANK64((uint64_t)lm[2])] = CO_SLOT_EDGE(64 + lane);
  }
  WAVE_SYNC();
  CO_PH(15);
  return b;
}

CO_DEV uint32_t co_create_node(CoWave &w, CoTree &t, uint64_t board, uint32_t meta_game, int depth, uint32_t parent,
                               uint32_t self_slot, int *res_out, int *n_out = (int *)0, uint32_t *lm_out = (uint32_t *)0) {
  uint32_t lm[3];
  int is_lines = co_legal_moves1(board, meta_game, lm);
  CO_PH(14);
  if (lm_out) {
    lm_out[0] = lm[0];
    lm_out[1] = lm[1];
    lm_out[2] = lm[2];
  }
  int n = co_popc32(lm[0]) + co_popc32(lm[1]) + co_popc32(lm[2]);
  int res = CO_RESULT_NONE;
  if (n == 0) res = is_lines ? CO_RESULT_LOSS : CO_RESULT_DRAW;
  *res_out = res;
  if (n_out) *n_out = n;
  return co_emit_node(w, t, board, meta_game, depth, parent, self_slot, lm, n, res);
}

CO_DEV void co_request(CoWave &w, uint64_t board, uint32_t meta, uint32_t leaf, int n_edges, const uint32_t lm[3], int D,
                       const uint32_t *path_slot) {
  int k = w.gc.n_pending;
  co_write_state(board, meta, w.req + (size_t)k * CO_STATE_STRIDE);
  CO_PH(17);
  uint32_t *pp = w.pend_path + (size_t)k * CO_PATH_MAX;
  const uint32_t pn = ((uint32_t)w.noise_words << 8) | (uint32_t)n_edges;
  w.noise_words += n_edges;
  FOR_LANES {
    if (lane == 0) {
      w.pend_leaf[k] = leaf;
      w.pend_depth[k] = D;
    }
    if (lane < 4) w.pend_n[4 * k + lane] = lane == 0 ? pn : lm[lane == 1 ? 0 : lane == 2 ? 1 : 2];
    if (lane <= D && lane < CO_PATH_MAX) pp[lane] = path_slot[lane];
    if (lane == 0 && w.pend_key) {
      const uint32_t pc = meta & 0x3FFFFu;
      const uint32_t rot = ((meta >> 18) & 1u) ? ((pc >> 9) | (pc << 9)) & 0x3FFFFu : pc;
      w.pend_key[k] = make_uint4((uint32_t)board, (uint32_t)(board >> 32), rot | 0x80000000u, 0u);
    }
  }
  WAVE_SYNC();
  w.gc.n_pending = k + 1;
  CO_PH(18);
}
```

Measured before the change: 10640.

## Add compile-time specialized training-mode MCTS step kernel

Templates the MCTS step path on a mode policy class and adds a CoModeTrain kernel where testing, analyse, trace, log, player-config and arena checks are compile-time constants. The host picks this kernel when the runtime parameters match plain training self-play. The aim is to drop dead branches, shrink code size and register pressure, and let the compiler fold the per-wave flags. The cost is a second kernel instantiation and a possible mismatch if the host predicate misses some flag.

```diff
diff --git a/corintho_ai_amd/csrc/kernels.h b/corintho_ai_amd/csrc/kernels.h
--- a/corintho_ai_amd/csrc/kernels.h
+++ b/corintho_ai_amd/csrc/kernels.h
@@ -17,6 +17,11 @@
   const int i = CO_BLOCK_IDX * CO_K3_WAVES + CO_K3_WAVE_IN_BLOCK;
   const int g = P.pool_lo + i;
   if (i < P.pool_n && g < P.num_games) co_mcts_step_wave(P, g);
+}
+CO_K3_BOUNDS CO_KERNEL co_k_mcts_step_train(EngineParams P) {
+  const int i = CO_BLOCK_IDX * CO_K3_WAVES + CO_K3_WAVE_IN_BLOCK;
+  const int g = P.pool_lo + i;
+  if (i < P.pool_n && g < P.num_games) co_mcts_step_wave<CoModeTrain>(P, g);
 }
 
 CO_DEV int co_game_active(const EngineParams &P, int g, const GameCtl &gc, int tp) {
diff --git a/corintho_ai_amd/csrc/pools.h b/corintho_ai_amd/csrc/pools.h
--- a/corintho_ai_amd/csrc/pools.h
+++ b/corintho_ai_amd/csrc/pools.h
@@ -26,8 +26,18 @@
   }
 };
 
+static bool co_params_train(const EngineParams &e) {
+#ifdef CO_K3_GENERAL_ONLY
+  return false;
+#else
+  return e.fused_pack == 1 && !e.testing && !e.analyse && !e.pcfg && !e.arena_state && e.to_play == -1 && !e.log &&
+         !(e.trace_on && e.trace);
+#endif
+}
+
 static void launch_mcts_step(const EngineParams &e, int n, rt_stream_t s) {
-  RT_LAUNCH(co_k_mcts_step, (n + CO_K3_WAVES - 1) / CO_K3_WAVES, CO_WAVE * CO_K3_WAVES, s, e);
+  if (co_params_train(e)) RT_LAUNCH(co_k_mcts_step_train, (n + CO_K3_WAVES - 1) / CO_K3_WAVES, CO_WAVE * CO_K3_WAVES, s, e);
+  else RT_LAUNCH(co_k_mcts_step, (n + CO_K3_WAVES - 1) / CO_K3_WAVES, CO_WAVE * CO_K3_WAVES, s, e);
 }
 
 struct CacheTable {
diff --git a/corintho_ai_amd/csrc/search_group.h b/corintho_ai_amd/csrc/search_group.h
--- a/corintho_ai_amd/csrc/search_group.h
+++ b/corintho_ai_amd/csrc/search_group.h
@@ -23,6 +23,7 @@
 #define CO_SBP(w, i, v) ((void)0)
 #endif
 
+template <class M = CoModeAny>
 CO_DEV int co_search_rows(CoWave &w, CoTree &t, CoRoot &rc, int m) {
   uint4 *A = t.A;
   WAVE_SHARED(uint32_t, sb_block, CO_SB * CO_SB_DEPTH);
@@ -632,7 +633,7 @@
     }
     CO_PH(15);
     CO_PROF_ADD(w, 24, (unsigned long long)nsel);
-    if (w.analyse) {
+    if (M::analyse(w)) {
       for (int j = 0; j < nsel; ++j) {
         const int D = WAVE_BCAST(leafD, 16 * j);
         FOR_LANES_HOT {
@@ -706,7 +707,7 @@
     const uint32_t none[3] = {0u, 0u, 0u};
     const uint32_t nb = co_emit_node(w, t, board, meta, depth, parent, child_slot, none, 0, res);
     if (nb != CO_NONE) {
-      if (w.analyse) {
+      if (M::analyse(w)) {
         FOR_LANES_HOT {
           if (lane < D) A[CO_NODE_INFO(pblock[lane])].z += 1u;
         }
diff --git a/corintho_ai_amd/csrc/search_iter.h b/corintho_ai_amd/csrc/search_iter.h
--- a/corintho_ai_amd/csrc/search_iter.h
+++ b/corintho_ai_amd/csrc/search_iter.h
@@ -26,11 +26,12 @@
   co_request(w, board, h0.z, root, (int)CO_META_NEDGES(h0.z), lm, 0, one_path);
 }
 
+template <class M = CoModeAny>
 CO_DEV int co_mc_do_iteration(CoWave &w, CoTree &t, const float *eval, const float *probs) {
   if (t.tc.root == CO_NONE) {
     int res;
-    const uint64_t b0 = w.analyse ? ((uint64_t)w.gc.pos_lo | ((uint64_t)w.gc.pos_hi << 32)) : 0ull;
-    uint32_t b = co_create_node(w, t, b0, w.analyse ? (w.gc.pos_meta & 0x7FFFFu) : CO_META_START, 0, CO_NONE, CO_NONE, &res);
+    const uint64_t b0 = M::analyse(w) ? ((uint64_t)w.gc.pos_lo | ((uint64_t)w.gc.pos_hi << 32)) : 0ull;
+    uint32_t b = co_create_node(w, t, b0, M::analyse(w) ? (w.gc.pos_meta & 0x7FFFFu) : CO_META_START, 0, CO_NONE, CO_NONE, &res);
     if (b == CO_NONE) return 0;
     t.tc.root = b;
     t.tc.searches_done = 1;
@@ -73,7 +74,7 @@
       if (w.max_searches - t.tc.searches_done < m) m = w.max_searches - t.tc.searches_done;
       if (m > cap) m = cap;
       if (m > 1 && (int)CO_META_NEDGES(rc.h0.z) <= CO_WAVE) {
-        const int r = co_search_rows(w, t, rc, m);
+        const int r = co_search_rows<M>(w, t, rc, m);
         w.gc.held |= 4;
         for (int i = 0; i < (r & 0xFF); ++i) pe -= pe >> 3;
         if (r & 0x300) {
@@ -86,7 +87,7 @@
     const int pending_before = w.gc.n_pending;
     CO_SBS(8, 1);
     CO_SBP(w, 6, 1);
-    co_search(w, t, rc);
+    co_search<M>(w, t, rc);
     w.gc.held |= 4;
     CO_PROF_ADD(w, 5, 1ull);
     if (!counted) {
diff --git a/corintho_ai_amd/csrc/search_move.h b/corintho_ai_amd/csrc/search_move.h
--- a/corintho_ai_amd/csrc/search_move.h
+++ b/corintho_ai_amd/csrc/search_move.h
@@ -115,6 +115,7 @@
   co_log_commit(w, at);
 }
 
+template <class M = CoModeAny>
 CO_COLD int co_choose_move(CoWave &w, CoTree &t, float *sample) {
   uint4 *A = t.A;
   uint32_t root = t.tc.root;
@@ -126,7 +127,7 @@
   int rres = co_slot_result(rs);
   uint64_t board = (uint64_t)h0.x | ((uint64_t)h0.y << 32);
   float *policy = sample ? sample + CO_GAME_STATE_SIZE : (float *)0;
-  if (!w.testing) {
+  if (!M::testing(w)) {
     WAVE_SHARED(float, srow, CO_STATE_STRIDE);
     co_write_state(board, h0.z, srow);
     WAVE_SYNC();
@@ -139,7 +140,7 @@
     WAVE_SYNC();
   }
   WAVE_SHARED(uint4, ch, CO_NUM_MOVES);
-  if (w.log) co_log_ply(w, t, ch);
+  if (M::log(w)) co_log_ply(w, t, ch);
   for (int base = 0; base < n; base += CO_WAVE) {
     FOR_LANES {
       int e = base + lane;
@@ -147,22 +148,22 @@
     }
   }
   WAVE_SYNC();
-  if (w.trace_on) {
-    co_trace_push(w, w.gc.to_play);
-    co_trace_push(w, (int)CO_META_DEPTH(h0.z));
-    co_trace_push(w, co_slot_visits(rs));
-    co_trace_push(w, rres);
-    co_trace_push(w, (int32_t)rs.y);
+  if (M::trace_on(w)) {
+    co_trace_push<M>(w, w.gc.to_play);
+    co_trace_push<M>(w, (int)CO_META_DEPTH(h0.z));
+    co_trace_push<M>(w, co_slot_visits(rs));
+    co_trace_push<M>(w, rres);
+    co_trace_push<M>(w, (int32_t)rs.y);
     int nc = 0;
     for (int e = 0; e < n; ++e) nc += ch[e].x != CO_NONE;
-    co_trace_push(w, nc);
+    co_trace_push<M>(w, nc);
     for (int e = 0; e < n; ++e) {
       if (ch[e].x == CO_NONE) continue;
-      co_trace_push(w, (int)CO_SLOT_MOVE(ch[e].z));
-      co_trace_push(w, co_slot_visits(ch[e]));
-      co_trace_push(w, (int32_t)ch[e].y);
-      co_trace_push(w, co_slot_result(ch[e]));
-      co_trace_push(w, co_slot_all_visited(ch[e]));
+      co_trace_push<M>(w, (int)CO_SLOT_MOVE(ch[e].z));
+      co_trace_push<M>(w, co_slot_visits(ch[e]));
+      co_trace_push<M>(w, (int32_t)ch[e].y);
+      co_trace_push<M>(w, co_slot_result(ch[e]));
+      co_trace_push<M>(w, co_slot_all_visited(ch[e]));
     }
   }
   int choice = 0;
@@ -195,7 +196,7 @@
         choice = (int)CO_SLOT_MOVE(ch[e].z);
       }
     }
-    if ((int)CO_META_DEPTH(h0.z) < 6 && !w.testing) {
+    if ((int)CO_META_DEPTH(h0.z) < 6 && !M::testing(w)) {
       int32_t visits = 0;
       for (int e = 0; e < n; ++e)
         if (ch[e].x != CO_NONE && !co_res_won(co_slot_result(ch[e]))) visits += co_slot_visits(ch[e]);
@@ -310,8 +311,9 @@
   return 1;
 }
 
+template <class M = CoModeAny>
 CO_DEV void co_use_player(CoWave &w, int p) {
-  if (!w.pc) return;
+  if (!M::pc(w)) return;
   w.max_searches = w.pc[p].max_searches;
   w.spe = w.pc[p].searches_per_eval;
   w.c_puct = w.pc[p].c_puct;
diff --git a/corintho_ai_amd/csrc/search_one.h b/corintho_ai_amd/csrc/search_one.h
--- a/corintho_ai_amd/csrc/search_one.h
+++ b/corintho_ai_amd/csrc/search_one.h
@@ -7,6 +7,7 @@
 #include "search_eval.h"
 #include "search_puct.h"
 
+template <class M = CoModeAny>
 CO_COLD2 void co_search(CoWave &w, CoTree &t, CoRoot &rc) {
   uint4 *A = t.A;
   WAVE_SHARED(uint32_t, path_block, CO_PATH_MAX);
@@ -101,7 +102,7 @@
       CO_PROF_ADD(w, 24, 1ull);
       uint32_t nb = co_create_node(w, t, board, meta, depth, cur, child_slot, &res, &leaf_n, leaf_lm);
       if (nb == CO_NONE) return;
-      if (w.analyse) {
+      if (M::analyse(w)) {
         FOR_LANES {
           if (lane <= D) A[CO_NODE_INFO(path_block[lane])].z += 1u;
         }
diff --git a/corintho_ai_amd/csrc/search_state.h b/corintho_ai_amd/csrc/search_state.h
--- a/corintho_ai_amd/csrc/search_state.h
+++ b/corintho_ai_amd/csrc/search_state.h
@@ -84,3 +84,39 @@
   float c_puct, epsilon;
   const PlayerCfg *pc;
 };
+
+#ifdef CO_EMU
+#define CO_MODE_Q static inline
+#else
+#define CO_MODE_Q static __device__ __forceinline__
+#endif
+struct CoModeAny {
+  static constexpr int train = 0;
+  CO_MODE_Q int testing(const CoWave &w) { return w.testing; }
+  CO_MODE_Q int analyse(const CoWave &w) { return w.analyse; }
+  CO_MODE_Q int force_choose(const CoWave &w) { return w.force_choose; }
+  CO_MODE_Q int trace_on(const CoWave &w) { return w.trace_on; }
+  CO_MODE_Q int32_t *log(const CoWave &w) { return w.log; }
+  CO_MODE_Q const PlayerCfg *pc(const CoWave &w) { return w.pc; }
+  CO_MODE_Q int testing(const EngineParams &P) { return P.testing; }
+  CO_MODE_Q int analyse(const EngineParams &P) { return P.analyse; }
+  CO_MODE_Q int fused_pack(const EngineParams &P) { return P.fused_pack; }
+  CO_MODE_Q const PlayerCfg *pcfg(const EngineParams &P) { return P.pcfg; }
+  CO_MODE_Q int32_t *arena_state(const EngineParams &P) { return P.arena_state; }
+  CO_MODE_Q int to_play(const EngineParams &P) { return P.to_play; }
+};
+struct CoModeTrain {
+  static constexpr int train = 1;
+  CO_MODE_Q int testing(const CoWave &) { return 0; }
+  CO_MODE_Q int analyse(const CoWave &) { return 0; }
+  CO_MODE_Q int force_choose(const CoWave &) { return 0; }
+  CO_MODE_Q int trace_on(const CoWave &) { return 0; }
+  CO_MODE_Q int32_t *log(const CoWave &) { return (int32_t *)0; }
+  CO_MODE_Q const PlayerCfg *pc(const CoWave &) { return (const PlayerCfg *)0; }
+  CO_MODE_Q int testing(const EngineParams &) { return 0; }
+  CO_MODE_Q int analyse(const EngineParams &) { return 0; }
+  CO_MODE_Q int fused_pack(const EngineParams &) { return 1; }
+  CO_MODE_Q const PlayerCfg *pcfg(const EngineParams &) { return (const PlayerCfg *)0; }
+  CO_MODE_Q int32_t *arena_state(const EngineParams &) { return (int32_t *)0; }
+  CO_MODE_Q int to_play(const EngineParams &) { return -1; }
+};
diff --git a/corintho_ai_amd/csrc/search_step.h b/corintho_ai_amd/csrc/search_step.h
--- a/corintho_ai_amd/csrc/search_step.h
+++ b/corintho_ai_amd/csrc/search_step.h
@@ -9,6 +9,7 @@
 #include "search_iter.h"
 #include "search_move.h"
 
+template <class M = CoModeAny>
 CO_DEV int co_game_step(CoWave &w, const float *eval, const float *probs) {
   const float *ev = eval, *pr = probs;
   if (w.gc.resume) {
@@ -16,11 +17,11 @@
     ev = pr = (const float *)0;
   }
   if (w.gc.held & 1) ev = pr = (const float *)0;
-  int skip_iteration = (w.pc && w.pc[w.gc.to_play].random)  || w.force_choose;
+  int skip_iteration = (M::pc(w) && M::pc(w)[w.gc.to_play].random)  || M::force_choose(w);
   int fresh_root = 0;
   for (;;) {
     if (!skip_iteration) {
-      int done = co_mc_do_iteration(w, w.me, ev, pr);
+      int done = co_mc_do_iteration<M>(w, w.me, ev, pr);
       if (w.gc.error) return 0;
       if (fresh_root) return done;
       if (!done) return 0;
@@ -32,22 +33,22 @@
     int choice, terminal, tres, depth;
     uint64_t board;
     uint32_t meta;
-    if (w.pc && w.pc[p].random) {
+    if (M::pc(w) && M::pc(w)[p].random) {
       board = (uint64_t)w.gc.pos_lo | ((uint64_t)w.gc.pos_hi << 32);
       meta = w.gc.pos_meta;
       uint32_t lm[3];
       co_legal_moves1(board, meta, lm);
       int n = co_popc32(lm[0]) + co_popc32(lm[1]) + co_popc32(lm[2]);
       choice = co_nth_move(lm, (int)co_uniform_below(w, (uint32_t)n));
-      co_trace_push(w, -2);
-      co_trace_push(w, choice);
+      co_trace_push<M>(w, -2);
+      co_trace_push<M>(w, choice);
       w.gc.plies++;
       co_do_move_lane(&board, &meta, choice);
       int lines = co_legal_moves1(board, meta, lm);
       terminal = (lm[0] | lm[1] | lm[2]) == 0u;
       tres = lines ? CO_RESULT_LOSS : CO_RESULT_DRAW;
       depth = w.gc.plies;
-      if (w.log) {
+      if (M::log(w)) {
         int at = w.log[0];
         co_log_put(w, at, 2);
         co_log_put(w, at, choice);
@@ -58,27 +59,27 @@
       }
     } else {
       CoTree &me = w.me;
-      if (!w.pc) {
+      if (!M::pc(w)) {
         uint4 rs = co_load_unit(me.A, co_load_unit(me.A, CO_NODE_INFO(me.tc.root)).x);
         if (co_res_known(co_slot_result(rs)) && w.gc.mate_turn == 0) w.gc.mate_turn = w.gc.n_samples + 1;
       }
       float *sample = (float *)0;
-      if (!w.testing) {
+      if (!M::testing(w)) {
         if (w.gc.n_samples >= CO_MAX_PLIES) {
           w.gc.error |= CO_ERR_TOO_MANY_PLIES;
           return 0;
         }
         sample = w.samples + (size_t)w.gc.n_samples * CO_SAMPLE_FLOATS;
       }
-      choice = co_choose_move(w, me, sample);
+      choice = co_choose_move<M>(w, me, sample);
       if (w.gc.error) return 0;
-      if (w.analyse) {
+      if (M::analyse(w)) {
         co_analyse_finish(w, me, choice);
         w.gc.plies++;
         return 1;
       }
-      if (!w.testing) w.gc.n_samples++;
-      co_trace_push(w, choice);
+      if (!M::testing(w)) w.gc.n_samples++;
+      co_trace_push<M>(w, choice);
       w.gc.plies++;
       uint4 h0 = co_load_unit(me.A, me.tc.root);
       uint4 nrs = co_load_unit(me.A, co_load_unit(me.A, CO_NODE_INFO(me.tc.root)).x);
@@ -87,7 +88,7 @@
       board = (uint64_t)h0.x | ((uint64_t)h0.y << 32);
       meta = h0.z;
       depth = (int)CO_META_DEPTH(h0.z);
-      if (w.log) {
+      if (M::log(w)) {
         int at = w.log[0];
         co_log_put(w, at, choice);
         co_log_put(w, at, (int32_t)h0.x);
@@ -96,7 +97,7 @@
         co_log_commit(w, at);
       }
     }
-    if (w.pc) {
+    if (M::pc(w)) {
       w.gc.pos_lo = (uint32_t)board;
       w.gc.pos_hi = (uint32_t)(board >> 32);
       w.gc.pos_meta = meta & 0x7FFFFu;
@@ -114,8 +115,8 @@
       w.me = w.opp;
       w.opp = tmp;
     }
-    co_use_player(w, 1 - p);
-    if (w.pc && w.pc[1 - p].random) {
+    co_use_player<M>(w, 1 - p);
+    if (M::pc(w) && M::pc(w)[1 - p].random) {
       skip_iteration = 1;
       continue;
     }
@@ -136,11 +137,12 @@
   }
 }
 
+template <class M = CoModeAny>
 CO_DEV int co_step_gate(const EngineParams &P, int g, const GameCtl &gc) {
   if (gc.done || gc.error) return 0;
-  const int tp = P.arena_state ? P.arena_state[CO_AS_MODEL] : P.to_play;
-  if (P.pcfg) {
-    if (tp != CO_TO_PLAY_EVERY_MODEL && P.pcfg[2 * g + gc.to_play].model_id != tp) return 0;
+  const int tp = M::arena_state(P) ? M::arena_state(P)[CO_AS_MODEL] : M::to_play(P);
+  if (M::pcfg(P)) {
+    if (tp != CO_TO_PLAY_EVERY_MODEL && M::pcfg(P)[2 * g + gc.to_play].model_id != tp) return 0;
   } else if (tp == 0 || tp == 1) {
     if (gc.to_play != (tp + gc.parity) % 2) return 0;
   } else if (P.stagger_div > 0) {
@@ -149,8 +151,9 @@
   return 1;
 }
 
+template <class M = CoModeAny>
 CO_DEV int co_step_row(const EngineParams &P, int g, const GameCtl &gc) {
-  return P.fused_pack ? gc.row_off : P.read_offset ? P.read_offset[g] : P.req_offset[g];
+  return M::fused_pack(P) ? gc.row_off : P.read_offset ? P.read_offset[g] : P.req_offset[g];
 }
 
 CO_DEV uint32_t co_cache_hash(uint32_t k0, uint32_t k1, uint32_t k2) {
@@ -238,8 +241,9 @@
 }
 
 
+template <class M = CoModeAny>
 CO_DEV void co_pool_housekeeping(const EngineParams &P, int g) {
-  if (P.fused_pack && g == P.pool_lo) {
+  if (M::fused_pack(P) && g == P.pool_lo) {
     FOR_LANES {
       if (lane == 0) {
         P.pack_counter[(P.iteration + 1) & 1] = 0ull;
@@ -272,13 +276,15 @@
 }
 
 #define CO_STEP_BUDGET_NONE (1 << 28)
+template <class M = CoModeAny>
 CO_DEV int co_step_budget(const EngineParams &P) {
-  if (!(P.fused_pack && !P.testing && !P.analyse && !P.pcfg)) return CO_STEP_BUDGET_NONE;
+  if (!(M::fused_pack(P) && !M::testing(P) && !M::analyse(P) && !M::pcfg(P))) return CO_STEP_BUDGET_NONE;
   int b = P.step_budget * CO_STEP_UNITS_PER_CONFIG_UNIT;
   if (P.step_budget == 0 && P.step_budget_k16 > 0 && P.work_counter) b = (int)(uint32_t)P.work_counter[CO_WC_BUDGET + ((P.iteration + 1) & 1)];
   return b > 0 ? b : CO_STEP_BUDGET_NONE;
 }
 
+template <class M = CoModeAny>
 CO_DEV void co_wave_init(const EngineParams &P, int g, const GameCtl &gc, const TreeCtl &tc0, const TreeCtl &tc1, CoWave &w) {
   w.g = g;
   w.gc = gc;
@@ -300,31 +306,38 @@
   w.pend_key = P.cache.hdr ? P.pend_key + (size_t)g * P.searches_per_eval : (uint4 *)0;
   w.noise_raw = P.noise_raw + (size_t)g * P.searches_per_eval * CO_NUM_MOVES;
   w.noise_words = (gc.held & 1) ? gc.noise_held : 0;
-  w.work = CO_STEP_START(co_step_budget(P));
+  w.work = CO_STEP_START(co_step_budget<M>(P));
   w.req = P.req + (size_t)g * P.searches_per_eval * CO_STATE_STRIDE;
   w.samples = P.samples ? P.samples + (size_t)gc.gid * CO_MAX_PLIES * CO_SAMPLE_FLOATS : (float *)0;
-  w.trace = P.trace ? P.trace + (size_t)gc.gid * CO_TRACE_CAP : (int32_t *)0;
-  w.log = (int32_t *)0;
-  if (P.log) {
-    const int rec = P.log_index ? P.log_index[gc.gid] : gc.gid < P.num_logged ? gc.gid : -1;
-    if (rec >= 0) w.log = P.log + (size_t)rec * CO_LOG_CAP;
+  if (!M::train) {
+    w.trace = P.trace ? P.trace + (size_t)gc.gid * CO_TRACE_CAP : (int32_t *)0;
+    w.log = (int32_t *)0;
+    if (P.log) {
+      const int rec = P.log_index ? P.log_index[gc.gid] : gc.gid < P.num_logged ? gc.gid : -1;
+      if (rec >= 0) w.log = P.log + (size_t)rec * CO_LOG_CAP;
+    }
   }
   w.prof = P.prof ? P.prof + (size_t)g * CO_NPROF : (unsigned long long *)0;
   w.max_searches = P.max_searches;
   w.spe = P.searches_per_eval;
-  w.testing = P.testing;
-  w.trace_on = P.trace_on && P.trace;
+  if (!M::train) {
+    w.testing = P.testing;
+    w.trace_on = P.trace_on && P.trace;
+  }
   w.defer_handover = P.defer_handover;
-  w.analyse = P.analyse;
-  w.force_choose = P.analyse && P.force_choose;
+  if (!M::train) {
+    w.analyse = P.analyse;
+    w.force_choose = P.analyse && P.force_choose;
+  }
   w.c_puct = P.c_puct;
   w.epsilon = P.epsilon;
-  w.pc = P.pcfg ? P.pcfg + 2 * g : (const PlayerCfg *)0;
-  co_use_player(w, gc.to_play);
+  if (!M::train) w.pc = P.pcfg ? P.pcfg + 2 * g : (const PlayerCfg *)0;
+  co_use_player<M>(w, gc.to_play);
   w.cval = P.cache.hdr ? P.cache.val : (const float *)0;
   w.csrc = P.cache.hdr ? P.pend_src + (size_t)g * P.searches_per_eval : (const int32_t *)0;
 }
 
+template <class M = CoModeAny>
 CO_COLD int co_slot_next_game(const EngineParams &P, CoWave &w) {
   w.gc.done = 1;
   if (!P.results) return 0;
@@ -357,19 +370,22 @@
   w.opp.tc.root = CO_NONE; w.opp.tc.searches_done = 0; w.opp.tc.units_used = 0u;
   w.noise_words = 0;
   w.samples = P.samples ? P.samples + (size_t)gid * CO_MAX_PLIES * CO_SAMPLE_FLOATS : (float *)0;
-  w.trace = P.trace ? P.trace + (size_t)gid * CO_TRACE_CAP : (int32_t *)0;
-  w.log = (int32_t *)0;
+  if (!M::train) {
+    w.trace = P.trace ? P.trace + (size_t)gid * CO_TRACE_CAP : (int32_t *)0;
+    w.log = (int32_t *)0;
+  }
   co_mt_seed(w.mt, P.seeds[gid]);
   w.mt_staged = 0;
   return 1;
 }
 
+template <class M = CoModeAny>
 CO_DEV void co_step_tail(const EngineParams &P, CoWave &w, int g, int done) {
-  const int packs = P.fused_pack && !w.gc.done && !w.gc.error;
+  const int packs = M::fused_pack(P) && !w.gc.done && !w.gc.error;
   unsigned long long old = 0ull;
   CO_PH_MEM(25);
   if (packs && P.work_counter) {
-    const int scans = CO_STEP_DONE(w, co_step_budget(P));
+    const int scans = CO_STEP_DONE(w, co_step_budget<M>(P));
     if (scans > 0) co_atomic_add_u64_noret(P.work_counter + P.iteration % 3, ((w.gc.held & 2) ? 0ull : 1ull << 32) | (unsigned long long)scans);
   }
   w.gc.held &= 1;
@@ -409,13 +425,14 @@
   }
 }
 
+template <class M = CoModeAny>
 CO_DEV void co_mcts_step_wave(const EngineParams &P, int g) {
-  co_pool_housekeeping(P, g);
+  co_pool_housekeeping<M>(P, g);
   GameCtl gc = P.games[g];
   const TreeCtl tc0 = P.trees[2 * g], tc1 = P.trees[2 * g + 1];
-  const int gate = co_step_gate(P, g, gc);
+  const int gate = co_step_gate<M>(P, g, gc);
   if (gate != 1) {
-    if (gate == 2 && P.fused_pack) co_atomic_add_u64(P.pack_counter + (P.iteration & 1), CO_PACK_ONE_RUNNING);
+    if (gate == 2 && M::fused_pack(P)) co_atomic_add_u64(P.pack_counter + (P.iteration & 1), CO_PACK_ONE_RUNNING);
     return;
   }
   CoWave w;
@@ -440,24 +457,24 @@
   for (int i = 0; i < CO_NPROF; ++i) w.pacc[i] = 0ull;
   w.tph = t_wave0;
 #endif
-  co_wave_init(P, g, gc, tc0, tc1, w);
+  co_wave_init<M>(P, g, gc, tc0, tc1, w);
   w.pre_n = 0;
   if (w.gc.n_pending > 0 && !(w.gc.held & 1)) co_pending_records(w, 0, w.gc.n_pending < CO_PRE ? w.gc.n_pending : CO_PRE);
   co_mt_stage_load(w.mt, w.mt_stage);
   w.mt_staged = 1;
   CO_PROF_ADD(w, 4, 1ull);
   CO_PH_MEM(22);
-  int off = co_step_row(P, g, gc);
+  int off = co_step_row<M>(P, g, gc);
   const float *step_eval = P.nn_eval + off, *step_probs = P.nn_probs + (size_t)off * CO_NUM_MOVES;
   int done;
   for (;;) {
-    done = co_game_step(w, step_eval, step_probs);
+    done = co_game_step<M>(w, step_eval, step_probs);
     if (!done) break;
-    if (!co_slot_next_game(P, w)) break;
+    if (!co_slot_next_game<M>(P, w)) break;
     step_eval = step_probs = (const float *)0;
   }
   CO_PH(20);
-  co_step_tail(P, w, g, done);
+  co_step_tail<M>(P, w, g, done);
   CO_PH_MEM(21);
 #if defined(CO_PROF) && !defined(CO_EMU)
   w.pacc[7] = CO_CLK() - t_wave0;
diff --git a/corintho_ai_amd/csrc/search_tree.h b/corintho_ai_amd/csrc/search_tree.h
--- a/corintho_ai_amd/csrc/search_tree.h
+++ b/corintho_ai_amd/csrc/search_tree.h
@@ -54,8 +54,9 @@
   WAVE_SYNC();
 }
 
+template <class M = CoModeAny>
 CO_DEV void co_trace_push(CoWave &w, int32_t v) {
-  if (!w.trace_on) return;
+  if (!M::trace_on(w)) return;
   if (w.gc.trace_len < CO_TRACE_CAP) {
     int at = w.gc.trace_len;
     FOR_LANES {
```

Result: no change. 10650 (median of 6 runs) (+0.1%).
